# Kamino666/video_features

Measured on NVIDIA H100. Metric: frames/sec CLIP-ViT-B/32 @224px, higher is better.
Workload: dtype f16

## Files before the change

### include/vfeat.h

```cpp
#ifndef VFEAT_H_
#define VFEAT_H_
#include <stddef.h>
#include <stdint.h>

#ifdef __cplusplus
extern "C" {
#endif

#define VF_OK 0
#define VF_ERR_INVALID 1
#define VF_ERR_CUDA 2
#define VF_ERR_NOMEM 3
#define VF_ERR_UNSUPPORTED 4

#define VF_ACT_NONE 0
#define VF_ACT_QUICKGELU 1
#define VF_ACT_RELU 2
#define VF_ACT_SIGMOID 3
#define VF_ACT_TANH 4
#define VF_ACT_LEAKY 5
#define VF_ACT_GELU 6

#define VF_FILTER_BILINEAR 2
#define VF_FILTER_BICUBIC 3

int vf_version(void);
const char* vf_last_error(void);

int vf_sample_indices(const char* method, int param, int64_t frame_cnt, double fps, int64_t* out_idx, int64_t cap,
                      int64_t* out_n);
int vf_shard_range(int64_t n_items, int n_parts, int part, int64_t* begin, int64_t* end);

int vf_resize_u8(const uint8_t* src, int n, int in_h, int in_w, uint8_t* dst, int out_h, int out_w, int filter,
                 uint8_t* tmp, void* stream);
int vf_resize_geometry(int in_h, int in_w, int size, int to_smaller_edge, int* out_h, int* out_w);

int vf_clip_normalize_u8(const uint8_t* src, int n, int src_h, int src_w, float* dst, void* stream);

int vf_gemm_f16(const void* A, int lda, const void* B, int ldb, int M, int N, int K, void* D, int ldd, int out_f32,
                const float* bias, const float* scale, int act, void* stream);
int vf_gemm_f16_accumulate(const void* A, int lda, const void* B, int ldb, int M, int N, int K, float* D, int ldd,
                           const float* bias, const float* scale, int act, void* stream);
int vf_gemm_f16_split(const void* A, int lda, const void* B, int ldb, int M, int N, int K, void* D, int ldd, int split_off,
                      const float* bias, const float* scale, int act, void* stream);
int vf_conv_gemm_f16(const void* X, int C, int64_t P, const void* Wt, int N, int ntaps, int k_per_tap, const int* tap_off,
                     int nsplit, uint64_t lo_mask, int row0, const int* region, void* D, int ldd, int out_f32, int split_off,
                     const float* bias, const float* scale, int act, void* stream);

int vf_gemm_profile(int enable);
int vf_gemm_profile_read(double* ms, int64_t* launches, double* executed_flops);

typedef struct vf_clip_layer_weights {
    const float *ln_1_w, *ln_1_b;
    const float *in_proj_w, *in_proj_b;
    const float *out_proj_w, *out_proj_b;
    const float *ln_2_w, *ln_2_b;
    const float *c_fc_w, *c_fc_b;
    const float *c_proj_w, *c_proj_b;
} vf_clip_layer_weights;

typedef struct vf_clip_weights {
    const float* conv1_w;
    const float* class_embedding;
    const float* positional_embedding;
    const float *ln_pre_w, *ln_pre_b, *ln_post_w, *ln_post_b;
    const float* proj;
    vf_clip_layer_weights layers[12];
} vf_clip_weights;

typedef struct vf_clip vf_clip_t;

int vf_clip_create(vf_clip_t** out, const vf_clip_weights* w, int device, int chunk_frames);
int vf_clip_create_vit(vf_clip_t** out, const vf_clip_weights* w, int device, int chunk_frames, int patch_size);
int vf_clip_destroy(vf_clip_t* h);
int vf_clip_encode_f32(vf_clip_t* h, const float* frames, int n, float* out, void* stream);
int vf_clip_encode_u8(vf_clip_t* h, const uint8_t* frames, int n, int src_h, int src_w, float* out, void* stream);
int vf_clip_encode_u8_host(vf_clip_t* h, const uint8_t* frames_host, int n, int src_h, int src_w, float* out_host,
                           void* stream);
int vf_clip_encode_u8_host_dev(vf_clip_t* h, const uint8_t* frames_host, int n, int src_h, int src_w, float* out_dev,
                               float* out_host, void* stream);

int vf_clip_encode_u8_host_async(vf_clip_t* h, const uint8_t* frames_host, int n, int src_h, int src_w, float* out_dev,
                                 float* out_host, void* stream, int64_t* ticket);
int vf_clip_wait(vf_clip_t* h, int64_t ticket);
int vf_clip_block_attention(vf_clip_t* h, int layer, const void* x, int n_frames, void* out, int fused, void* stream);
int vf_clip_debug_embed_f32(vf_clip_t* h, const float* frames, int n, float* x_out, void* stream);
int vf_clip_debug_embed_u8(vf_clip_t* h, const uint8_t* frames, int n, int src_h, int src_w, float* x_out, void* stream);
int vf_clip_debug_blocks(vf_clip_t* h, float* x, int n_frames, int layer_begin, int layer_end, void* stream);
int vf_clip_debug_head(vf_clip_t* h, const float* x, int n_frames, float* out, void* stream);
int64_t vf_clip_launch_count(const vf_clip_t* h);
int vf_clip_profile(vf_clip_t* h, int enable);
int vf_clip_profile_read(vf_clip_t* h, double* gemm_ms, int64_t* gemm_launches, double* gemm_flops);
int vf_clip_profile_categories(const vf_clip_t* h, double* ms4);

#define VF_I3D_UNITS 57
typedef struct vf_conv_unit {
    const float* w;
    const float *bn_w, *bn_b, *bn_mean, *bn_var;
    int cout, cin, k;
} vf_conv_unit;
typedef struct vf_i3d_weights {
    vf_conv_unit units[VF_I3D_UNITS];
} vf_i3d_weights;
typedef struct vf_i3d vf_i3d_t;

int vf_i3d_create(vf_i3d_t** out, const vf_i3d_weights* w, int in_channels, int device, int max_stacks, int max_T);
int vf_i3d_destroy(vf_i3d_t* h);
int vf_i3d_forward_f32(vf_i3d_t* h, const float* clips, int n, int T, float* out, void* stream);
int vf_i3d_forward_u8(vf_i3d_t* h, const uint8_t* frames, int n, int T, int Hr, int Wr, float* out, void* stream);
int vf_i3d_forward_u8_strided(vf_i3d_t* h, const uint8_t* frames, int n, int T, int64_t stack_stride, int Hr, int Wr,
                              float* out, void* stream);
int vf_i3d_forward_flow(vf_i3d_t* h, const float* flow, int n, int T, int H, int W, float* out, void* stream);
int vf_i3d_read_stage(vf_i3d_t* h, int stage, float* out, int64_t capacity, int* dims5, void* stream);
int64_t vf_i3d_launch_count(const vf_i3d_t* h);
int vf_i3d_conv(const vf_i3d_t* h, int index, int* geom, uint64_t* lo_mask, void* w, float* scale, float* bias);
int vf_i3d_debug_mixed(vf_i3d_t* h, int block, const void* x_pairs, int n, int T, void* out_pairs, void* stream);

typedef struct vf_named_tensor {
    const char* name;
    const float* data;
    int64_t numel;
} vf_named_tensor;
typedef struct vf_raft vf_raft_t;

int vf_raft_create(vf_raft_t** out, const vf_named_tensor* tensors, int n_tensors, int device, int max_frames, int max_h,
                   int max_w);
int vf_raft_destroy(vf_raft_t* h);
int vf_raft_flow(vf_raft_t* h, const void* frames, int is_u8, int chw_layout, int n_frames, int Hs, int Ws, int iters,
                 int unpad, float* out, void* stream);
int vf_raft_padded_size(int Hs, int Ws, int* H, int* W);
int vf_raft_debug_read(vf_raft_t* h, int what, float* out, int64_t capacity, int* dims4, void* stream);
int64_t vf_raft_launch_count(const vf_raft_t* h);
int vf_raft_conv(const vf_raft_t* h, int index, int* geom, uint64_t* lo_mask, void* w, float* scale, float* bias);

typedef struct vf_pwc vf_pwc_t;

int vf_pwc_create(vf_pwc_t** out, const vf_named_tensor* tensors, int n_tensors, int device, int max_frames, int max_h,
                  int max_w);
int vf_pwc_destroy(vf_pwc_t* h);
int vf_pwc_flow(vf_pwc_t* h, const void* frames, int is_u8, int chw_layout, int n_frames, int Hs, int Ws, float* out,
                void* stream);
int vf_pwc_debug_read(vf_pwc_t* h, int what, int level, float* out, int64_t capacity, int* dims4, void* stream);
int64_t vf_pwc_launch_count(const vf_pwc_t* h);
int vf_pwc_conv(const vf_pwc_t* h, int index, int* geom, uint64_t* lo_mask, void* w, float* scale, float* bias);

typedef struct vf_resnet vf_resnet_t;

int vf_resnet_create(vf_resnet_t** out, const vf_named_tensor* tensors, int n_tensors, int depth, int device, int max_frames);
int vf_resnet_destroy(vf_resnet_t* h);
int vf_resnet_forward_f32(vf_resnet_t* h, const float* frames, int n, float* out, void* stream);
int vf_resnet_forward_u8(vf_resnet_t* h, const uint8_t* frames, int n, int Hr, int Wr, float* out, void* stream);
int vf_resnet_read_stage(vf_resnet_t* h, int stage, float* out, int64_t capacity, int* dims4, void* stream);
int64_t vf_resnet_launch_count(const vf_resnet_t* h);
int vf_resnet_conv(const vf_resnet_t* h, int index, int* geom, uint64_t* lo_mask, void* w, float* scale, float* bias);

typedef struct vf_r21d vf_r21d_t;

int vf_r21d_create(vf_r21d_t** out, const vf_named_tensor* tensors, int n_tensors, int device, int max_clips, int max_T);
int vf_r21d_create2(vf_r21d_t** out, const vf_named_tensor* tensors, int n_tensors, int device, int max_clips, int max_T,
                    double bn_eps);
int vf_r21d_destroy(vf_r21d_t* h);
int vf_r21d_forward_f32(vf_r21d_t* h, const float* clips, int n, int T, float* out, void* stream);
int vf_r21d_forward_u8(vf_r21d_t* h, const uint8_t* frames, int n_frames, int H, int W, const int* starts, int n, int T,
                       float* out, void* stream);
int vf_r21d_read_stage(vf_r21d_t* h, int stage, float* out, int64_t capacity, int* dims5, void* stream);
int64_t vf_r21d_launch_count(const vf_r21d_t* h);
int vf_r21d_conv(const vf_r21d_t* h, int index, int* geom, uint64_t* lo_mask, void* w, float* scale, float* bias);

typedef struct vf_clip_rn vf_clip_rn_t;

int vf_clip_rn_create(vf_clip_rn_t** out, const vf_named_tensor* tensors, int n_tensors, int device, int max_frames);
int vf_clip_rn_destroy(vf_clip_rn_t* h);
int vf_clip_rn_info(const vf_clip_rn_t* h, int* info);
int vf_clip_rn_encode_f32(vf_clip_rn_t* h, const float* frames, int n, float* out, void* stream);
int vf_clip_rn_encode_u8(vf_clip_rn_t* h, const uint8_t* frames, int n, int H, int W, float* out, void* stream);
int vf_clip_rn_read_stage(vf_clip_rn_t* h, int stage, float* out, int64_t capacity, int* dims4, void* stream);
int64_t vf_clip_rn_launch_count(const vf_clip_rn_t* h);
int vf_clip_rn_read_pairs(vf_clip_rn_t* h, int stage, void* out, int64_t capacity, void* stream);
int vf_clip_rn_conv(const vf_clip_rn_t* h, int index, int* geom, uint64_t* lo_mask, void* w, float* scale, float* bias);
int vf_clip_rn_debug_block(vf_clip_rn_t* h, int block, const void* x_pairs, int n, void* out_pairs, void* branch_out,
                           void* shortcut_out, void* stream);
int vf_clip_rn_debug_attnpool(vf_clip_rn_t* h, const void* x_pairs, int n, float* features, void* stream);
int vf_clip_rn_debug_attnpool_read(vf_clip_rn_t* h, int what, void* out, int64_t capacity, void* stream);
int vf_debug_clip_rn_attention(const float* kv, const float* q, int n, int T, int E, void* out_pairs, void* stream);

typedef struct vf_clip_vitl vf_clip_vitl_t;

int vf_clip_vitl_create(vf_clip_vitl_t** out, const vf_named_tensor* tensors, int n_tensors, int device, int max_frames);
int vf_clip_vitl_destroy(vf_clip_vitl_t* h);
int vf_clip_vitl_info(const vf_clip_vitl_t* h, int* info);
int vf_clip_vitl_encode_f32(vf_clip_vitl_t* h, const float* frames, int n, float* out, void* stream);
int vf_clip_vitl_encode_u8(vf_clip_vitl_t* h, const uint8_t* frames, int n, int H, int W, float* out, void* stream);
int vf_clip_vitl_debug_embed_f32(vf_clip_vitl_t* h, const float* frames, int n, float* x_out, void* stream);
int vf_clip_vitl_debug_embed_u8(vf_clip_vitl_t* h, const uint8_t* frames, int n, int H, int W, float* x_out,
                                void* stream);
int vf_clip_vitl_debug_blocks(vf_clip_vitl_t* h, float* x, int n, int layer_begin, int layer_end, void* stream);
int vf_clip_vitl_debug_head(vf_clip_vitl_t* h, const float* x, int n, float* out, void* stream);
int vf_clip_vitl_attention(vf_clip_vitl_t* h, const void* qkv, int n_frames, int tokens, void* out, void* stream);
int64_t vf_clip_vitl_launch_count(const vf_clip_vitl_t* h);

typedef struct vf_vggish vf_vggish_t;

int vf_vggish_create(vf_vggish_t** out, const vf_named_tensor* tensors, int n_tensors, const double* hann,
                     const double* mel, const double* interp_win, int n_win, int num_table, int device,
                     int max_examples);
int vf_vggish_destroy(vf_vggish_t* h);
int vf_vggish_forward_pcm16(vf_vggish_t* h, const int16_t* samples, int64_t n_samples, int channels, int sample_rate,
                            float* out, int64_t capacity, int64_t* n_out, void* stream);
int vf_vggish_forward_logmel_f32(vf_vggish_t* h, const float* examples, int n, float* out, void* stream);
int vf_vggish_read_stage(vf_vggish_t* h, int stage, void* out, int64_t capacity, int* dims4, void* stream);
int64_t vf_vggish_launch_count(const vf_vggish_t* h);
int vf_vggish_conv(const vf_vggish_t* h, int index, int* geom, uint64_t* lo_mask, void* w, float* scale, float* bias);
int vf_vggish_time_register(int sample_rate, int64_t t0, int64_t count, double* out);

typedef struct vf_s3d vf_s3d_t;

int vf_s3d_create(vf_s3d_t** out, const vf_named_tensor* tensors, int n_tensors, int device, int max_clips, int max_T);
int vf_s3d_destroy(vf_s3d_t* h);
int vf_s3d_forward_f32(vf_s3d_t* h, const float* clips, int n, int T, float* out, void* stream);
int vf_s3d_forward_u8(vf_s3d_t* h, const uint8_t* frames, int n_frames, int H, int W, const int* starts, int n, int T,
                      float* out, void* stream);
int vf_s3d_read_stage(vf_s3d_t* h, int stage, float* out, int64_t capacity, int* dims5, void* stream);
int64_t vf_s3d_launch_count(const vf_s3d_t* h);
int vf_s3d_conv(const vf_s3d_t* h, int index, int* geom, uint64_t* lo_mask, void* w, float* scale, float* bias);
int vf_s3d_debug_mixed(vf_s3d_t* h, int block, const void* x_pairs, int n, int T, void* out_pairs, void* stream);

#define VF_POOL_GENERAL 0
#define VF_POOL_FAST 1
#define VF_POOL_SAME3 2
int vf_debug_maxpool3d(const void* in, const int* vol_in, void* out, const int* vol_out, int C, const int* k,
                       const int* s, const int* p, int* path, void* stream);
int vf_debug_i3d_head(const void* in, const int* vol, int C, float* out, void* stream);

typedef struct vf_swin3d vf_swin3d_t;

int vf_swin3d_create(vf_swin3d_t** out, const vf_named_tensor* tensors, int n_tensors, int device, int max_clips,
                     int max_T);
int vf_swin3d_destroy(vf_swin3d_t* h);
int vf_swin3d_info(const vf_swin3d_t* h, int* info);
int vf_swin3d_forward_f32(vf_swin3d_t* h, const float* clips, int n, int T, float* out, void* stream);
int vf_swin3d_forward_u8(vf_swin3d_t* h, const uint8_t* frames, int n_frames, int H, int W, const int* starts, int n,
                         int T, float* out, void* stream);
int vf_swin3d_read_stage(vf_swin3d_t* h, int stage, float* out, int64_t capacity, int* dims5, void* stream);
int vf_swin3d_attention(const void* qkv, const float* bias_qkv, const float* table, int n, int Tq, int H, int W, int C,
                        int shifted, void* out, void* stream);
int64_t vf_swin3d_launch_count(const vf_swin3d_t* h);

typedef struct vf_mvit vf_mvit_t;

int vf_mvit_create(vf_mvit_t** out, const vf_named_tensor* tensors, int n_tensors, int device, int max_clips);
int vf_mvit_destroy(vf_mvit_t* h);
int vf_mvit_info(const vf_mvit_t* h, int* info);
int vf_mvit_forward_f32(vf_mvit_t* h, const float* clips, int n, int T, float* out, void* stream);
int vf_mvit_forward_u8(vf_mvit_t* h, const uint8_t* frames, int n_frames, int H, int W, const int* starts, int n, int T,
                       float* out, void* stream);
int vf_mvit_read_stage(vf_mvit_t* h, int stage, float* out, int64_t capacity, int* dims3, void* stream);
int vf_mvit_attention(const void* q, int ldq, const void* k, const void* v, const float* rel_h, const float* rel_w,
                      const float* rel_t, int n, int heads, const int* q_thw, const int* k_thw, int rel, int resid,
                      void* out, void* stream);
int vf_mvit_head_pool(const void* src, int ld_src, int n, int heads, int T, int H, int W, int stride,
                      const float* weight, const float* gamma, const float* beta, void* dst, void* stream);
int vf_mvit_skip_pool(const float* x, int n, int C, int T, int H, int W, float* y, void* stream);
int64_t vf_mvit_launch_count(const vf_mvit_t* h);

typedef struct vf_clip_text vf_clip_text_t;

int vf_clip_text_create(vf_clip_text_t** out, const vf_named_tensor* tensors, int n_tensors, int device, int max_rows);
int vf_clip_text_destroy(vf_clip_text_t* h);
int vf_clip_text_info(const vf_clip_text_t* h, int* info);
int vf_clip_text_encode(vf_clip_text_t* h, const int32_t* tokens, int n, float* out, void* stream);
int vf_clip_text_blocks(vf_clip_text_t* h, float* x, int n, int L, int first, int count, void* stream);
int vf_clip_text_attention(const void* qkv, int n, int L, int heads, void* out, void* stream);
int vf_l2_normalize_rows(const float* x, int n, int C, float* out, void* stream);
int64_t vf_clip_text_launch_count(const vf_clip_text_t* h);

typedef struct vf_dinov2 vf_dinov2_t;

int vf_dinov2_create(vf_dinov2_t** out, const vf_named_tensor* tensors, int n_tensors, int device, int max_frames);
int vf_dinov2_destroy(vf_dinov2_t* h);
int vf_dinov2_info(const vf_dinov2_t* h, int* info);
int vf_dinov2_encode_f32(vf_dinov2_t* h, const float* frames, int n, float* out, void* stream);
int vf_dinov2_encode_u8(vf_dinov2_t* h, const uint8_t* frames, int n, int H, int W, float* out, void* stream);
int vf_dinov2_debug_embed_f32(vf_dinov2_t* h, const float* frames, int n, float* x_out, void* stream);
int vf_dinov2_debug_embed_u8(vf_dinov2_t* h, const uint8_t* frames, int n, int H, int W, float* x_out, void* stream);
int vf_dinov2_debug_blocks(vf_dinov2_t* h, float* x, int n, int layer_begin, int layer_end, void* stream);
int vf_dinov2_debug_head(vf_dinov2_t* h, const float* x, int n, float* out, void* stream);
int vf_dinov2_swiglu(const float* ab, int rows, int hidden, void* out, void* stream);
int vf_dinov2_attention(const void* qkv, int n, int S, int heads, void* out, void* stream);
int64_t vf_dinov2_launch_count(const vf_dinov2_t* h);

typedef struct vf_videomae vf_videomae_t;

int vf_videomae_create(vf_videomae_t** out, const vf_named_tensor* tensors, int n_tensors, const float* config,
                       int device, int max_clips);
int vf_videomae_destroy(vf_videomae_t* h);
int vf_videomae_info(const vf_videomae_t* h, int* info);
int vf_videomae_forward_f32(vf_videomae_t* h, const float* clips, int n, int T, float* out, void* stream);
int vf_videomae_forward_u8(vf_videomae_t* h, const uint8_t* frames, int n_frames, int H, int W, const int* starts, int n,
                           int T, float* out, void* stream);
int vf_videomae_debug_tubelets_u8(vf_videomae_t* h, const uint8_t* frames, int n_frames, int H, int W,
                                  const int* starts, int n, void* tubelets, void* stream);
int vf_videomae_debug_tubelets_f32(vf_videomae_t* h, const float* clips, int n, void* tubelets, void* stream);
int vf_videomae_debug_embed(vf_videomae_t* h, const void* tubelets, int n, float* x_out, void* stream);
int vf_videomae_debug_blocks(vf_videomae_t* h, float* x, int n, int layer_begin, int layer_end, void* stream);
int vf_videomae_debug_head(vf_videomae_t* h, const float* x, int n, float* out, void* stream);
int vf_videomae_debug_drop_lo(vf_videomae_t* h);
int vf_videomae_attention(const void* qkv, int n, int S, int heads, void* out, void* stream);
int64_t vf_videomae_launch_count(const vf_videomae_t* h);

typedef struct vf_head vf_head_t;

int vf_head_create(vf_head_t** out, const float* weight, const float* bias, int n_classes, int n_features, int device);
int vf_head_destroy(vf_head_t* h);
int vf_head_info(const vf_head_t* h, int* n_classes, int* n_features);
int vf_head_forward(vf_head_t* h, const float* feats, int n, int n_features, float* logits, float* probs, int k,
                    int32_t* top_idx, float* top_logit, float* top_prob, void* stream);

#ifdef __cplusplus
}
#endif
#endif
```

### video_features_b200/_lib.py

```python
from __future__ import annotations

import ctypes as C
import os
import threading

_HERE = os.path.dirname(os.path.abspath(__file__))
LIB_PATH = os.environ.get("VF_LIBVFEAT") or os.path.join(_HERE, "libvfeat.so")

VF_OK = 0
VF_ACT_NONE, VF_ACT_QUICKGELU, VF_ACT_RELU, VF_ACT_SIGMOID, VF_ACT_TANH, VF_ACT_LEAKY = 0, 1, 2, 3, 4, 5
VF_ACT_GELU = 6
VF_FILTER_BILINEAR, VF_FILTER_BICUBIC = 2, 3
VF_POOL_GENERAL, VF_POOL_FAST, VF_POOL_SAME3 = 0, 1, 2


class VfError(RuntimeError):
    def __init__(self, code: int, text: str):
        super().__init__(f"libvfeat error {code}: {text}")
        self.code = code


class ClipLayerWeights(C.Structure):
    _fields_ = [(n, C.POINTER(C.c_float)) for n in (
        "ln_1_w", "ln_1_b", "in_proj_w", "in_proj_b", "out_proj_w", "out_proj_b",
        "ln_2_w", "ln_2_b", "c_fc_w", "c_fc_b", "c_proj_w", "c_proj_b")]


class ClipWeights(C.Structure):
    _fields_ = [(n, C.POINTER(C.c_float)) for n in (
        "conv1_w", "class_embedding", "positional_embedding",
        "ln_pre_w", "ln_pre_b", "ln_post_w", "ln_post_b", "proj")] + [("layers", ClipLayerWeights * 12)]


class ConvUnitW(C.Structure):
    _fields_ = [("w", C.POINTER(C.c_float)), ("bn_w", C.POINTER(C.c_float)), ("bn_b", C.POINTER(C.c_float)),
                ("bn_mean", C.POINTER(C.c_float)), ("bn_var", C.POINTER(C.c_float)),
                ("cout", C.c_int), ("cin", C.c_int), ("k", C.c_int)]


I3D_UNITS = 57


class I3DWeights(C.Structure):
    _fields_ = [("units", ConvUnitW * I3D_UNITS)]


class NamedTensor(C.Structure):
    _fields_ = [("name", C.c_char_p), ("data", C.POINTER(C.c_float)), ("numel", C.c_int64)]


def named_tensors(state_dict):
    import numpy as np
    import torch
    items = state_dict.items() if hasattr(state_dict, "items") else state_dict
    items = [(k, v) for k, v in items if torch.is_tensor(v) and v.dtype.is_floating_point]
    keep = []
    arr = (NamedTensor * max(len(items), 1))()
    for i, (k, v) in enumerate(items):
        a = np.ascontiguousarray(v.detach().to("cpu", torch.float32).numpy())
        nm = k.encode()
        keep.append((a, nm))
        arr[i].name = nm
        arr[i].data = a.ctypes.data_as(C.POINTER(C.c_float))
        arr[i].numel = a.size
    return arr, len(items), keep


_lock = threading.Lock()
_lib = None

SIGNATURES = {
    "vf_version": (C.c_int, []),
    "vf_last_error": (C.c_char_p, []),
    "vf_sample_indices": (C.c_int, [C.c_char_p, C.c_int, C.c_int64, C.c_double, C.POINTER(C.c_int64), C.c_int64,
                                    C.POINTER(C.c_int64)]),
    "vf_shard_range": (C.c_int, [C.c_int64, C.c_int, C.c_int, C.POINTER(C.c_int64), C.POINTER(C.c_int64)]),
    "vf_resize_u8": (C.c_int, [C.c_void_p, C.c_int, C.c_int, C.c_int, C.c_void_p, C.c_int, C.c_int, C.c_int,
                               C.c_void_p, C.c_void_p]),
    "vf_resize_geometry": (C.c_int, [C.c_int, C.c_int, C.c_int, C.c_int, C.POINTER(C.c_int), C.POINTER(C.c_int)]),
    "vf_clip_normalize_u8": (C.c_int, [C.c_void_p, C.c_int, C.c_int, C.c_int, C.c_void_p, C.c_void_p]),
    "vf_gemm_f16": (C.c_int, [C.c_void_p, C.c_int, C.c_void_p, C.c_int, C.c_int, C.c_int, C.c_int, C.c_void_p,
                              C.c_int, C.c_int, C.c_void_p, C.c_void_p, C.c_int, C.c_void_p]),
    "vf_gemm_f16_accumulate": (C.c_int, [C.c_void_p, C.c_int, C.c_void_p, C.c_int, C.c_int, C.c_int, C.c_int, C.c_void_p,
                                         C.c_int, C.c_void_p, C.c_void_p, C.c_int, C.c_void_p]),
    "vf_gemm_f16_split": (C.c_int, [C.c_void_p, C.c_int, C.c_void_p, C.c_int, C.c_int, C.c_int, C.c_int, C.c_void_p,
                                    C.c_int, C.c_int, C.c_void_p, C.c_void_p, C.c_int, C.c_void_p]),
    "vf_conv_gemm_f16": (C.c_int, [C.c_void_p, C.c_int, C.c_int64, C.c_void_p, C.c_int, C.c_int, C.c_int,
                                   C.POINTER(C.c_int), C.c_int, C.c_uint64, C.c_int, C.POINTER(C.c_int), C.c_void_p,
                                   C.c_int, C.c_int, C.c_int, C.c_void_p, C.c_void_p, C.c_int, C.c_void_p]),
    "vf_gemm_profile": (C.c_int, [C.c_int]),
    "vf_gemm_profile_read": (C.c_int, [C.POINTER(C.c_double), C.POINTER(C.c_int64), C.POINTER(C.c_double)]),
    "vf_clip_create": (C.c_int, [C.POINTER(C.c_void_p), C.POINTER(ClipWeights), C.c_int, C.c_int]),
    "vf_clip_create_vit": (C.c_int, [C.POINTER(C.c_void_p), C.POINTER(ClipWeights), C.c_int, C.c_int, C.c_int]),
    "vf_clip_destroy": (C.c_int, [C.c_void_p]),
    "vf_clip_encode_f32": (C.c_int, [C.c_void_p, C.c_void_p, C.c_int, C.c_void_p, C.c_void_p]),
    "vf_clip_encode_u8": (C.c_int, [C.c_void_p, C.c_void_p, C.c_int, C.c_int, C.c_int, C.c_void_p, C.c_void_p]),
    "vf_clip_encode_u8_host": (C.c_int, [C.c_void_p, C.c_void_p, C.c_int, C.c_int, C.c_int, C.c_void_p, C.c_void_p]),
    "vf_clip_encode_u8_host_dev": (C.c_int, [C.c_void_p, C.c_void_p, C.c_int, C.c_int, C.c_int, C.c_void_p, C.c_void_p,
                                             C.c_void_p]),
    "vf_clip_encode_u8_host_async": (C.c_int, [C.c_void_p, C.c_void_p, C.c_int, C.c_int, C.c_int, C.c_void_p, C.c_void_p,
                                               C.c_void_p, C.POINTER(C.c_int64)]),
    "vf_clip_wait": (C.c_int, [C.c_void_p, C.c_int64]),
    "vf_clip_block_attention": (C.c_int, [C.c_void_p, C.c_int, C.c_void_p, C.c_int, C.c_void_p, C.c_int, C.c_void_p]),
    "vf_clip_debug_embed_f32": (C.c_int, [C.c_void_p, C.c_void_p, C.c_int, C.c_void_p, C.c_void_p]),
    "vf_clip_debug_embed_u8": (C.c_int, [C.c_void_p, C.c_void_p, C.c_int, C.c_int, C.c_int, C.c_void_p, C.c_void_p]),
    "vf_clip_debug_blocks": (C.c_int, [C.c_void_p, C.c_void_p, C.c_int, C.c_int, C.c_int, C.c_void_p]),
    "vf_clip_debug_head": (C.c_int, [C.c_void_p, C.c_void_p, C.c_int, C.c_void_p, C.c_void_p]),
    "vf_clip_launch_count": (C.c_int64, [C.c_void_p]),
    "vf_i3d_create": (C.c_int, [C.POINTER(C.c_void_p), C.POINTER(I3DWeights), C.c_int, C.c_int, C.c_int, C.c_int]),
    "vf_i3d_destroy": (C.c_int, [C.c_void_p]),
    "vf_i3d_forward_f32": (C.c_int, [C.c_void_p, C.c_void_p, C.c_int, C.c_int, C.c_void_p, C.c_void_p]),
    "vf_i3d_forward_u8": (C.c_int, [C.c_void_p, C.c_void_p, C.c_int, C.c_int, C.c_int, C.c_int, C.c_void_p, C.c_void_p]),
    "vf_i3d_forward_u8_strided": (C.c_int, [C.c_void_p, C.c_void_p, C.c_int, C.c_int, C.c_int64, C.c_int, C.c_int, C.c_void_p,
                                            C.c_void_p]),
    "vf_i3d_forward_flow": (C.c_int, [C.c_void_p, C.c_void_p, C.c_int, C.c_int, C.c_int, C.c_int, C.c_void_p, C.c_void_p]),
    "vf_i3d_read_stage": (C.c_int, [C.c_void_p, C.c_int, C.c_void_p, C.c_int64, C.POINTER(C.c_int), C.c_void_p]),
    "vf_i3d_launch_count": (C.c_int64, [C.c_void_p]),
    "vf_i3d_conv": (C.c_int, [C.c_void_p, C.c_int, C.POINTER(C.c_int), C.POINTER(C.c_uint64), C.c_void_p, C.c_void_p,
                              C.c_void_p]),
    "vf_i3d_debug_mixed": (C.c_int, [C.c_void_p, C.c_int, C.c_void_p, C.c_int, C.c_int, C.c_void_p, C.c_void_p]),
    "vf_raft_create": (C.c_int, [C.POINTER(C.c_void_p), C.POINTER(NamedTensor), C.c_int, C.c_int, C.c_int, C.c_int, C.c_int]),
    "vf_raft_destroy": (C.c_int, [C.c_void_p]),
    "vf_raft_flow": (C.c_int, [C.c_void_p, C.c_void_p, C.c_int, C.c_int, C.c_int, C.c_int, C.c_int, C.c_int, C.c_int,
                               C.c_void_p, C.c_void_p]),
    "vf_raft_padded_size": (C.c_int, [C.c_int, C.c_int, C.POINTER(C.c_int), C.POINTER(C.c_int)]),
    "vf_raft_debug_read": (C.c_int, [C.c_void_p, C.c_int, C.c_void_p, C.c_int64, C.POINTER(C.c_int), C.c_void_p]),
    "vf_raft_launch_count": (C.c_int64, [C.c_void_p]),
    "vf_raft_conv": (C.c_int, [C.c_void_p, C.c_int, C.POINTER(C.c_int), C.POINTER(C.c_uint64), C.c_void_p, C.c_void_p,
                               C.c_void_p]),
    "vf_pwc_create": (C.c_int, [C.POINTER(C.c_void_p), C.POINTER(NamedTensor), C.c_int, C.c_int, C.c_int, C.c_int, C.c_int]),
    "vf_pwc_destroy": (C.c_int, [C.c_void_p]),
    "vf_pwc_flow": (C.c_int, [C.c_void_p, C.c_void_p, C.c_int, C.c_int, C.c_int, C.c_int, C.c_int, C.c_void_p,
                              C.c_void_p]),
    "vf_pwc_debug_read": (C.c_int, [C.c_void_p, C.c_int, C.c_int, C.c_void_p, C.c_int64, C.POINTER(C.c_int), C.c_void_p]),
    "vf_pwc_launch_count": (C.c_int64, [C.c_void_p]),
    "vf_pwc_conv": (C.c_int, [C.c_void_p, C.c_int, C.POINTER(C.c_int), C.POINTER(C.c_uint64), C.c_void_p, C.c_void_p,
                              C.c_void_p]),
    "vf_resnet_create": (C.c_int, [C.POINTER(C.c_void_p), C.POINTER(NamedTensor), C.c_int, C.c_int, C.c_int, C.c_int]),
    "vf_resnet_destroy": (C.c_int, [C.c_void_p]),
    "vf_resnet_forward_f32": (C.c_int, [C.c_void_p, C.c_void_p, C.c_int, C.c_void_p, C.c_void_p]),
    "vf_resnet_forward_u8": (C.c_int, [C.c_void_p, C.c_void_p, C.c_int, C.c_int, C.c_int, C.c_void_p, C.c_void_p]),
    "vf_resnet_read_stage": (C.c_int, [C.c_void_p, C.c_int, C.c_void_p, C.c_int64, C.POINTER(C.c_int), C.c_void_p]),
    "vf_resnet_launch_count": (C.c_int64, [C.c_void_p]),
    "vf_resnet_conv": (C.c_int, [C.c_void_p, C.c_int, C.POINTER(C.c_int), C.POINTER(C.c_uint64), C.c_void_p,
                                 C.c_void_p, C.c_void_p]),
    "vf_r21d_create": (C.c_int, [C.POINTER(C.c_void_p), C.POINTER(NamedTensor), C.c_int, C.c_int, C.c_int, C.c_int]),
    "vf_r21d_create2": (C.c_int, [C.POINTER(C.c_void_p), C.POINTER(NamedTensor), C.c_int, C.c_int, C.c_int, C.c_int,
                                  C.c_double]),
    "vf_r21d_destroy": (C.c_int, [C.c_void_p]),
    "vf_r21d_forward_f32": (C.c_int, [C.c_void_p, C.c_void_p, C.c_int, C.c_int, C.c_void_p, C.c_void_p]),
    "vf_r21d_forward_u8": (C.c_int, [C.c_void_p, C.c_void_p, C.c_int, C.c_int, C.c_int, C.POINTER(C.c_int), C.c_int,
                                     C.c_int, C.c_void_p, C.c_void_p]),
    "vf_r21d_read_stage": (C.c_int, [C.c_void_p, C.c_int, C.c_void_p, C.c_int64, C.POINTER(C.c_int), C.c_void_p]),
    "vf_r21d_launch_count": (C.c_int64, [C.c_void_p]),
    "vf_r21d_conv": (C.c_int, [C.c_void_p, C.c_int, C.POINTER(C.c_int), C.POINTER(C.c_uint64), C.c_void_p,
                               C.c_void_p, C.c_void_p]),
    "vf_s3d_create": (C.c_int, [C.POINTER(C.c_void_p), C.POINTER(NamedTensor), C.c_int, C.c_int, C.c_int, C.c_int]),
    "vf_s3d_destroy": (C.c_int, [C.c_void_p]),
    "vf_s3d_forward_f32": (C.c_int, [C.c_void_p, C.c_void_p, C.c_int, C.c_int, C.c_void_p, C.c_void_p]),
    "vf_s3d_forward_u8": (C.c_int, [C.c_void_p, C.c_void_p, C.c_int, C.c_int, C.c_int, C.POINTER(C.c_int), C.c_int,
                                    C.c_int, C.c_void_p, C.c_void_p]),
    "vf_s3d_read_stage": (C.c_int, [C.c_void_p, C.c_int, C.c_void_p, C.c_int64, C.POINTER(C.c_int), C.c_void_p]),
    "vf_s3d_launch_count": (C.c_int64, [C.c_void_p]),
    "vf_s3d_conv": (C.c_int, [C.c_void_p, C.c_int, C.POINTER(C.c_int), C.POINTER(C.c_uint64), C.c_void_p,
                              C.c_void_p, C.c_void_p]),
    "vf_s3d_debug_mixed": (C.c_int, [C.c_void_p, C.c_int, C.c_void_p, C.c_int, C.c_int, C.c_void_p, C.c_void_p]),
    "vf_debug_maxpool3d": (C.c_int, [C.c_void_p, C.POINTER(C.c_int), C.c_void_p, C.POINTER(C.c_int), C.c_int,
                                     C.POINTER(C.c_int), C.POINTER(C.c_int), C.POINTER(C.c_int), C.POINTER(C.c_int),
                                     C.c_void_p]),
    "vf_debug_i3d_head": (C.c_int, [C.c_void_p, C.POINTER(C.c_int), C.c_int, C.c_void_p, C.c_void_p]),
    "vf_clip_rn_create": (C.c_int, [C.POINTER(C.c_void_p), C.POINTER(NamedTensor), C.c_int, C.c_int, C.c_int]),
    "vf_clip_rn_destroy": (C.c_int, [C.c_void_p]),
    "vf_clip_rn_info": (C.c_int, [C.c_void_p, C.POINTER(C.c_int)]),
    "vf_clip_rn_encode_f32": (C.c_int, [C.c_void_p, C.c_void_p, C.c_int, C.c_void_p, C.c_void_p]),
    "vf_clip_rn_encode_u8": (C.c_int, [C.c_void_p, C.c_void_p, C.c_int, C.c_int, C.c_int, C.c_void_p, C.c_void_p]),
    "vf_clip_rn_read_stage": (C.c_int, [C.c_void_p, C.c_int, C.c_void_p, C.c_int64, C.POINTER(C.c_int), C.c_void_p]),
    "vf_clip_rn_launch_count": (C.c_int64, [C.c_void_p]),
    "vf_clip_rn_conv": (C.c_int, [C.c_void_p, C.c_int, C.POINTER(C.c_int), C.POINTER(C.c_uint64), C.c_void_p,
                                  C.c_void_p, C.c_void_p]),
    "vf_clip_rn_read_pairs": (C.c_int, [C.c_void_p, C.c_int, C.c_void_p, C.c_int64, C.c_void_p]),
    "vf_clip_rn_debug_block": (C.c_int, [C.c_void_p, C.c_int, C.c_void_p, C.c_int, C.c_void_p, C.c_void_p, C.c_void_p,
                                         C.c_void_p]),
    "vf_clip_rn_debug_attnpool": (C.c_int, [C.c_void_p, C.c_void_p, C.c_int, C.c_void_p, C.c_void_p]),
    "vf_clip_rn_debug_attnpool_read": (C.c_int, [C.c_void_p, C.c_int, C.c_void_p, C.c_int64, C.c_void_p]),
    "vf_debug_clip_rn_attention": (C.c_int, [C.c_void_p, C.c_void_p, C.c_int, C.c_int, C.c_int, C.c_void_p,
                                             C.c_void_p]),
    "vf_swin3d_create": (C.c_int, [C.POINTER(C.c_void_p), C.POINTER(NamedTensor), C.c_int, C.c_int, C.c_int, C.c_int]),
    "vf_swin3d_destroy": (C.c_int, [C.c_void_p]),
    "vf_swin3d_info": (C.c_int, [C.c_void_p, C.POINTER(C.c_int)]),
    "vf_swin3d_forward_f32": (C.c_int, [C.c_void_p, C.c_void_p, C.c_int, C.c_int, C.c_void_p, C.c_void_p]),
    "vf_swin3d_forward_u8": (C.c_int, [C.c_void_p, C.c_void_p, C.c_int, C.c_int, C.c_int, C.POINTER(C.c_int), C.c_int,
                                       C.c_int, C.c_void_p, C.c_void_p]),
    "vf_swin3d_read_stage": (C.c_int, [C.c_void_p, C.c_int, C.c_void_p, C.c_int64, C.POINTER(C.c_int), C.c_void_p]),
    "vf_swin3d_attention": (C.c_int, [C.c_void_p, C.c_void_p, C.c_void_p, C.c_int, C.c_int, C.c_int, C.c_int, C.c_int,
                                      C.c_int, C.c_void_p, C.c_void_p]),
    "vf_swin3d_launch_count": (C.c_int64, [C.c_void_p]),
    "vf_mvit_create": (C.c_int, [C.POINTER(C.c_void_p), C.POINTER(NamedTensor), C.c_int, C.c_int, C.c_int]),
    "vf_mvit_destroy": (C.c_int, [C.c_void_p]),
    "vf_mvit_info": (C.c_int, [C.c_void_p, C.POINTER(C.c_int)]),
    "vf_mvit_forward_f32": (C.c_int, [C.c_void_p, C.c_void_p, C.c_int, C.c_int, C.c_void_p, C.c_void_p]),
    "vf_mvit_forward_u8": (C.c_int, [C.c_void_p, C.c_void_p, C.c_int, C.c_int, C.c_int, C.POINTER(C.c_int), C.c_int,
                                     C.c_int, C.c_void_p, C.c_void_p]),
    "vf_mvit_read_stage": (C.c_int, [C.c_void_p, C.c_int, C.c_void_p, C.c_int64, C.POINTER(C.c_int), C.c_void_p]),
    "vf_mvit_attention": (C.c_int, [C.c_void_p, C.c_int, C.c_void_p, C.c_void_p, C.c_void_p, C.c_void_p, C.c_void_p,
                                    C.c_int, C.c_int, C.POINTER(C.c_int), C.POINTER(C.c_int), C.c_int, C.c_int,
                                    C.c_void_p, C.c_void_p]),
    "vf_mvit_head_pool": (C.c_int, [C.c_void_p, C.c_int, C.c_int, C.c_int, C.c_int, C.c_int, C.c_int, C.c_int,
                                    C.c_void_p, C.c_void_p, C.c_void_p, C.c_void_p, C.c_void_p]),
    "vf_mvit_skip_pool": (C.c_int, [C.c_void_p, C.c_int, C.c_int, C.c_int, C.c_int, C.c_int, C.c_void_p, C.c_void_p]),
    "vf_mvit_launch_count": (C.c_int64, [C.c_void_p]),
    "vf_clip_vitl_create": (C.c_int, [C.POINTER(C.c_void_p), C.POINTER(NamedTensor), C.c_int, C.c_int, C.c_int]),
    "vf_clip_vitl_destroy": (C.c_int, [C.c_void_p]),
    "vf_clip_vitl_info": (C.c_int, [C.c_void_p, C.POINTER(C.c_int)]),
    "vf_clip_vitl_encode_f32": (C.c_int, [C.c_void_p, C.c_void_p, C.c_int, C.c_void_p, C.c_void_p]),
    "vf_clip_vitl_encode_u8": (C.c_int, [C.c_void_p, C.c_void_p, C.c_int, C.c_int, C.c_int, C.c_void_p, C.c_void_p]),
    "vf_clip_vitl_debug_embed_f32": (C.c_int, [C.c_void_p, C.c_void_p, C.c_int, C.c_void_p, C.c_void_p]),
    "vf_clip_vitl_debug_embed_u8": (C.c_int, [C.c_void_p, C.c_void_p, C.c_int, C.c_int, C.c_int, C.c_void_p,
                                              C.c_void_p]),
    "vf_clip_vitl_debug_blocks": (C.c_int, [C.c_void_p, C.c_void_p, C.c_int, C.c_int, C.c_int, C.c_void_p]),
    "vf_clip_vitl_debug_head": (C.c_int, [C.c_void_p, C.c_void_p, C.c_int, C.c_void_p, C.c_void_p]),
    "vf_clip_vitl_attention": (C.c_int, [C.c_void_p, C.c_void_p, C.c_int, C.c_int, C.c_void_p, C.c_void_p]),
    "vf_clip_vitl_launch_count": (C.c_int64, [C.c_void_p]),
    "vf_vggish_create": (C.c_int, [C.POINTER(C.c_void_p), C.POINTER(NamedTensor), C.c_int, C.c_void_p, C.c_void_p,
                                   C.c_void_p, C.c_int, C.c_int, C.c_int, C.c_int]),
    "vf_vggish_destroy": (C.c_int, [C.c_void_p]),
    "vf_vggish_forward_pcm16": (C.c_int, [C.c_void_p, C.c_void_p, C.c_int64, C.c_int, C.c_int, C.c_void_p, C.c_int64,
                                          C.POINTER(C.c_int64), C.c_void_p]),
    "vf_vggish_forward_logmel_f32": (C.c_int, [C.c_void_p, C.c_void_p, C.c_int, C.c_void_p, C.c_void_p]),
    "vf_vggish_read_stage": (C.c_int, [C.c_void_p, C.c_int, C.c_void_p, C.c_int64, C.POINTER(C.c_int), C.c_void_p]),
    "vf_vggish_launch_count": (C.c_int64, [C.c_void_p]),
    "vf_vggish_conv": (C.c_int, [C.c_void_p, C.c_int, C.POINTER(C.c_int), C.POINTER(C.c_uint64), C.c_void_p,
                                 C.c_void_p, C.c_void_p]),
    "vf_vggish_time_register": (C.c_int, [C.c_int, C.c_int64, C.c_int64, C.c_void_p]),
    "vf_clip_text_create": (C.c_int, [C.POINTER(C.c_void_p), C.POINTER(NamedTensor), C.c_int, C.c_int, C.c_int]),
    "vf_clip_text_destroy": (C.c_int, [C.c_void_p]),
    "vf_clip_text_info": (C.c_int, [C.c_void_p, C.POINTER(C.c_int)]),
    "vf_clip_text_encode": (C.c_int, [C.c_void_p, C.c_void_p, C.c_int, C.c_void_p, C.c_void_p]),
    "vf_clip_text_blocks": (C.c_int, [C.c_void_p, C.c_void_p, C.c_int, C.c_int, C.c_int, C.c_int, C.c_void_p]),
    "vf_clip_text_attention": (C.c_int, [C.c_void_p, C.c_int, C.c_int, C.c_int, C.c_void_p, C.c_void_p]),
    "vf_l2_normalize_rows": (C.c_int, [C.c_void_p, C.c_int, C.c_int, C.c_void_p, C.c_void_p]),
    "vf_clip_text_launch_count": (C.c_int64, [C.c_void_p]),
    "vf_dinov2_create": (C.c_int, [C.POINTER(C.c_void_p), C.POINTER(NamedTensor), C.c_int, C.c_int, C.c_int]),
    "vf_dinov2_destroy": (C.c_int, [C.c_void_p]),
    "vf_dinov2_info": (C.c_int, [C.c_void_p, C.POINTER(C.c_int)]),
    "vf_dinov2_encode_f32": (C.c_int, [C.c_void_p, C.c_void_p, C.c_int, C.c_void_p, C.c_void_p]),
    "vf_dinov2_encode_u8": (C.c_int, [C.c_void_p, C.c_void_p, C.c_int, C.c_int, C.c_int, C.c_void_p, C.c_void_p]),
    "vf_dinov2_debug_embed_f32": (C.c_int, [C.c_void_p, C.c_void_p, C.c_int, C.c_void_p, C.c_void_p]),
    "vf_dinov2_debug_embed_u8": (C.c_int, [C.c_void_p, C.c_void_p, C.c_int, C.c_int, C.c_int, C.c_void_p, C.c_void_p]),
    "vf_dinov2_debug_blocks": (C.c_int, [C.c_void_p, C.c_void_p, C.c_int, C.c_int, C.c_int, C.c_void_p]),
    "vf_dinov2_debug_head": (C.c_int, [C.c_void_p, C.c_void_p, C.c_int, C.c_void_p, C.c_void_p]),
    "vf_dinov2_swiglu": (C.c_int, [C.c_void_p, C.c_int, C.c_int, C.c_void_p, C.c_void_p]),
    "vf_dinov2_attention": (C.c_int, [C.c_void_p, C.c_int, C.c_int, C.c_int, C.c_void_p, C.c_void_p]),
    "vf_dinov2_launch_count": (C.c_int64, [C.c_void_p]),
    "vf_videomae_create": (C.c_int, [C.POINTER(C.c_void_p), C.POINTER(NamedTensor), C.c_int, C.POINTER(C.c_float),
                                     C.c_int, C.c_int]),
    "vf_videomae_destroy": (C.c_int, [C.c_void_p]),
    "vf_videomae_info": (C.c_int, [C.c_void_p, C.POINTER(C.c_int)]),
    "vf_videomae_forward_f32": (C.c_int, [C.c_void_p, C.c_void_p, C.c_int, C.c_int, C.c_void_p, C.c_void_p]),
    "vf_videomae_forward_u8": (C.c_int, [C.c_void_p, C.c_void_p, C.c_int, C.c_int, C.c_int, C.POINTER(C.c_int), C.c_int,
                                         C.c_int, C.c_void_p, C.c_void_p]),
    "vf_videomae_debug_tubelets_u8": (C.c_int, [C.c_void_p, C.c_void_p, C.c_int, C.c_int, C.c_int, C.POINTER(C.c_int),
                                                C.c_int, C.c_void_p, C.c_void_p]),
    "vf_videomae_debug_tubelets_f32": (C.c_int, [C.c_void_p, C.c_void_p, C.c_int, C.c_void_p, C.c_void_p]),
    "vf_videomae_debug_embed": (C.c_int, [C.c_void_p, C.c_void_p, C.c_int, C.c_void_p, C.c_void_p]),
    "vf_videomae_debug_blocks": (C.c_int, [C.c_void_p, C.c_void_p, C.c_int, C.c_int, C.c_int, C.c_void_p]),
    "vf_videomae_debug_head": (C.c_int, [C.c_void_p, C.c_void_p, C.c_int, C.c_void_p, C.c_void_p]),
    "vf_videomae_debug_drop_lo": (C.c_int, [C.c_void_p]),
    "vf_videomae_attention": (C.c_int, [C.c_void_p, C.c_int, C.c_int, C.c_int, C.c_void_p, C.c_void_p]),
    "vf_videomae_launch_count": (C.c_int64, [C.c_void_p]),
    "vf_head_create": (C.c_int, [C.POINTER(C.c_void_p), C.c_void_p, C.c_void_p, C.c_int, C.c_int, C.c_int]),
    "vf_head_destroy": (C.c_int, [C.c_void_p]),
    "vf_head_info": (C.c_int, [C.c_void_p, C.POINTER(C.c_int), C.POINTER(C.c_int)]),
    "vf_head_forward": (C.c_int, [C.c_void_p, C.c_void_p, C.c_int, C.c_int, C.c_void_p, C.c_void_p, C.c_int, C.c_void_p,
                                  C.c_void_p, C.c_void_p, C.c_void_p]),
    "vf_clip_profile": (C.c_int, [C.c_void_p, C.c_int]),
    "vf_clip_profile_categories": (C.c_int, [C.c_void_p, C.POINTER(C.c_double)]),
    "vf_clip_profile_read": (C.c_int, [C.c_void_p, C.POINTER(C.c_double), C.POINTER(C.c_int64),
                                       C.POINTER(C.c_double)]),
}


def lib() -> C.CDLL:
    global _lib
    if _lib is None:
        with _lock:
            if _lib is None:
                if not os.path.exists(LIB_PATH):
                    raise FileNotFoundError(
                        f"{LIB_PATH} not found: build the CUDA extension first (__graft_entry__.build()). "
                        "There is no CPU fallback.")
                l = C.CDLL(LIB_PATH)
                for name, (res, args) in SIGNATURES.items():
                    fn = getattr(l, name)
                    fn.restype = res
                    fn.argtypes = args
                _lib = l
    return _lib


def check(status: int) -> None:
    if status != VF_OK:
        raise VfError(status, lib().vf_last_error().decode("utf-8", "replace"))


def read_conv(fn, handle, index: int, device):
    import torch
    geom = (C.c_int * 15)()
    mask = C.c_uint64()
    check(fn(handle, index, geom, C.byref(mask), None, None, None))
    n_out, ntaps, kpt = geom[0], geom[1], geom[2]
    w = torch.empty((n_out, 2 * ntaps * kpt), dtype=torch.float16, device=device)
    scale = torch.empty(n_out, dtype=torch.float32, device=device)
    bias = torch.empty(n_out, dtype=torch.float32, device=device)
    check(fn(handle, index, geom, C.byref(mask), w.data_ptr(), scale.data_ptr(), bias.data_ptr()))
    shifts = [tuple(geom[3 + 3 * j:6 + 3 * j]) for j in range(ntaps)]
    return dict(n_out=n_out, ntaps=ntaps, k_per_tap=kpt, shifts=shifts, lo_mask=mask.value, w=w, scale=scale, bias=bias)


MIXED_SIDE = (28, 28, 14, 14, 14, 14, 14, 7, 7)
MIXED_WIDTHS = ((192, 64, 128, 32, 32), (256, 128, 192, 96, 64), (480, 192, 208, 48, 64), (512, 160, 224, 64, 64),
                (512, 128, 256, 64, 64), (512, 112, 288, 64, 64), (528, 256, 320, 128, 128), (832, 256, 320, 128, 128),
                (832, 384, 384, 128, 128))


def debug_mixed(fn, handle, block: int, x, device):
    import torch
    if not 0 <= block < len(MIXED_SIDE):
        raise ValueError(f"Mixed block {block} outside 0 .. {len(MIXED_SIDE) - 1}")
    S, cin, cout = MIXED_SIDE[block], MIXED_WIDTHS[block][0], sum(MIXED_WIDTHS[block][1:])
    if x.dtype != torch.float16 or x.dim() != 5 or tuple(x.shape[2:]) != (S + 2, S + 2, 2 * cin) or x.shape[1] < 3:
        raise ValueError(f"block {block} takes an fp16 pair volume (n, T + 2, {S + 2}, {S + 2}, {2 * cin}), T >= 1; "
                         f"got {x.dtype} {tuple(x.shape)}")
    if x.device != torch.device(device):
        raise ValueError(f"the volume is on {x.device}, the engine on {device}")
    x = x.contiguous()
    out = torch.empty(tuple(x.shape[:4]) + (2 * cout,), dtype=torch.float16, device=device)
    with torch.cuda.device(device):
        check(fn(handle, block, x.data_ptr(), x.shape[0], x.shape[1] - 2, out.data_ptr(),
                 torch.cuda.current_stream().cuda_stream))
    return out


def debug_maxpool3d(x, vol_in, vol_out, channels: int, k, s, p):
    import torch
    assert x.dtype == torch.float16 and x.is_cuda
    assert x.numel() == vol_in[0] * vol_in[1] * vol_in[2] * vol_in[3] * 2 * channels, (x.shape, vol_in, channels)
    x = x.contiguous()
    out = torch.empty(tuple(vol_out[:4]) + (2 * channels,), dtype=torch.float16, device=x.device)
    path = C.c_int(-1)
    with torch.cuda.device(x.device):
        check(lib().vf_debug_maxpool3d(x.data_ptr(), (C.c_int * 10)(*vol_in), out.data_ptr(), (C.c_int * 10)(*vol_out),
                                       channels, (C.c_int * 3)(*k), (C.c_int * 3)(*s), (C.c_int * 3)(*p), C.byref(path),
                                       torch.cuda.current_stream().cuda_stream))
    return out, path.value


def debug_i3d_head(x, vol, channels: int):
    import torch
    assert x.dtype == torch.float16 and x.is_cuda
    assert x.numel() == vol[0] * vol[1] * vol[2] * vol[3] * 2 * channels, (x.shape, vol, channels)
    x = x.contiguous()
    out = torch.empty((vol[0], channels), dtype=torch.float32, device=x.device)
    with torch.cuda.device(x.device):
        check(lib().vf_debug_i3d_head(x.data_ptr(), (C.c_int * 10)(*vol), channels, out.data_ptr(),
                                      torch.cuda.current_stream().cuda_stream))
    return out


def debug_clip_rn_attention(kv, q):
    import torch
    if kv.dtype != torch.float32 or q.dtype != torch.float32 or kv.dim() != 3 or q.dim() != 2:
        raise ValueError(f"kv (n, T, 2E) and q (n, E) fp32; got {kv.dtype} {tuple(kv.shape)}, {q.dtype} {tuple(q.shape)}")
    n, T, E2 = kv.shape
    if E2 % 2 or tuple(q.shape) != (n, E2 // 2):
        raise ValueError(f"kv {tuple(kv.shape)} and q {tuple(q.shape)} do not agree on (n, E)")
    if not kv.is_cuda or q.device != kv.device:
        raise ValueError(f"kv on {kv.device}, q on {q.device}: both must be on one CUDA device")
    kv, q = kv.contiguous(), q.contiguous()
    out = torch.empty((n, E2), dtype=torch.float16, device=kv.device)
    with torch.cuda.device(kv.device):
        check(lib().vf_debug_clip_rn_attention(kv.data_ptr(), q.data_ptr(), n, T, E2 // 2, out.data_ptr(),
                                               torch.cuda.current_stream().cuda_stream))
    return out


def read_split_conv(fn, handle, index: int, device):
    import torch
    geom = (C.c_int * 196)()
    mask = C.c_uint64()
    check(fn(handle, index, geom, C.byref(mask), None, None, None))
    n_out, ntaps, kpt, nsplit = geom[0], geom[1], geom[2], geom[3]
    w = torch.empty((n_out, nsplit * ntaps * kpt), dtype=torch.float16, device=device)
    scale = torch.empty(n_out, dtype=torch.float32, device=device)
    bias = torch.empty(n_out, dtype=torch.float32, device=device)
    check(fn(handle, index, geom, C.byref(mask), w.data_ptr(), scale.data_ptr(), bias.data_ptr()))
    shifts = [tuple(geom[4 + 3 * j:7 + 3 * j]) for j in range(ntaps)]
    return dict(n_out=n_out, ntaps=ntaps, k_per_tap=kpt, nsplit=nsplit, shifts=shifts, lo_mask=mask.value, w=w,
                scale=scale, bias=bias)
```

### video_features_b200/csrc/gemm.cu

```cuda
#include "gemm_kernel.cuh"

namespace vf {

extern template int launch_bn<1, false, true>(GEMM_LAUNCH_ARGS);
extern template int launch_bn<1, true, true>(GEMM_LAUNCH_ARGS);
extern template int launch_bn<1, false, false>(GEMM_LAUNCH_ARGS);
extern template int launch_bn<1, true, false>(GEMM_LAUNCH_ARGS);
extern template int launch_bn<2, false, false>(GEMM_LAUNCH_ARGS);
extern template int launch_bn<2, true, false>(GEMM_LAUNCH_ARGS);

namespace {

typedef CUresult (*EncodeTiledFn)(CUtensorMap*, CUtensorMapDataType, cuuint32_t, void*, const cuuint64_t*,
                                  const cuuint64_t*, const cuuint32_t*, const cuuint32_t*, CUtensorMapInterleave,
                                  CUtensorMapSwizzle, CUtensorMapL2promotion, CUtensorMapFloatOOBfill);

EncodeTiledFn get_encode_tiled() {
    static EncodeTiledFn fn = nullptr;
    if (fn) return fn;
    void* p = nullptr;
    cudaDriverEntryPointQueryResult q;
    if (cudaGetDriverEntryPoint("cuTensorMapEncodeTiled", &p, cudaEnableDefault, &q) != cudaSuccess ||
        q != cudaDriverEntryPointSuccess)
        return nullptr;
    fn = reinterpret_cast<EncodeTiledFn>(p);
    return fn;
}

}

int device_sm_count() {
    static std::atomic<int> sms[64];
    int dev = 0;
    if (cudaGetDevice(&dev) != cudaSuccess || dev < 0 || dev >= 64) return 132;
    int v = sms[dev].load(std::memory_order_relaxed);
    if (v == 0) {
        if (cudaDeviceGetAttribute(&v, cudaDevAttrMultiProcessorCount, dev) != cudaSuccess || v <= 0) v = 132;
        sms[dev].store(v, std::memory_order_relaxed);
    }
    return v;
}

int make_tmap_2d(CUtensorMap* out, const void* base, int elem_bytes, uint64_t rows, uint64_t cols,
                 uint64_t row_pitch_bytes, uint32_t box_rows, uint32_t box_cols) {
    EncodeTiledFn enc = get_encode_tiled();
    if (!enc) return fail(VF_ERR_CUDA, "cuTensorMapEncodeTiled entry point unavailable (no CUDA driver?)");
    if ((reinterpret_cast<uintptr_t>(base) & 15) || (row_pitch_bytes & 15))
        return fail(VF_ERR_INVALID, "TMA operand must be 16-byte aligned with a 16-byte multiple row pitch");
    if (box_cols * uint32_t(elem_bytes) != 128) return fail(VF_ERR_INVALID, "TMA box rows must be 128 bytes");
    const CUtensorMapDataType dt = elem_bytes == 2 ? CU_TENSOR_MAP_DATA_TYPE_FLOAT16 : CU_TENSOR_MAP_DATA_TYPE_FLOAT32;
    cuuint64_t dims[2] = {cols, rows};
    cuuint64_t strides[1] = {row_pitch_bytes};
    cuuint32_t box[2] = {box_cols, box_rows};
    cuuint32_t estr[2] = {1, 1};
    CUresult r = enc(out, dt, 2, const_cast<void*>(base), dims, strides, box, estr, CU_TENSOR_MAP_INTERLEAVE_NONE,
                     CU_TENSOR_MAP_SWIZZLE_128B, CU_TENSOR_MAP_L2_PROMOTION_L2_256B, CU_TENSOR_MAP_FLOAT_OOB_FILL_NONE);
    if (r != CUDA_SUCCESS) return fail(VF_ERR_CUDA, "cuTensorMapEncodeTiled failed with CUresult %d", int(r));
    return VF_OK;
}

struct GemmProf {
    bool on = false;
    std::vector<cudaEvent_t> ev;
    size_t used = 0;
    double flops = 0.0;
};
static thread_local GemmProf g_prof;

template <bool PP>
static int run_gemm_launch(const CUtensorMap& tmA, const CUtensorMap& tmB, const CUtensorMap& tmD,
                           const CUtensorMap& tmD2, int bn, const GemmEpi& ep, int M, int N, const ConvGeom& cg,
                           cudaStream_t stream) {
    const bool split = ep.split_off > 0 && !ep.out_f32;
    if constexpr (!PP) {
        if (cg.nsplit == 2)
            return split ? launch_bn<2, true, PP>(tmA, tmB, tmD, tmD2, bn, ep, M, N, cg, stream)
                         : launch_bn<2, false, PP>(tmA, tmB, tmD, tmD2, bn, ep, M, N, cg, stream);
    }
    return split ? launch_bn<1, true, PP>(tmA, tmB, tmD, tmD2, bn, ep, M, N, cg, stream)
                 : launch_bn<1, false, PP>(tmA, tmB, tmD, tmD2, bn, ep, M, N, cg, stream);
}

static int run_gemm(const CUtensorMap& tmA, bool pp, const __half* B, int ldb, int64_t Ktot, int M, int N,
                    const ConvGeom& cg, const GemmEpi& ep, cudaStream_t stream) {
    if (!ep.out) return fail(VF_ERR_INVALID, "gemm: null output");
    if (reinterpret_cast<uintptr_t>(ep.out) & 15) return fail(VF_ERR_INVALID, "gemm: output must be 16-byte aligned");
    if (ep.accumulate && !ep.out_f32) return fail(VF_ERR_INVALID, "gemm: accumulate needs fp32 output");
    if (N % 8) return fail(VF_ERR_INVALID, "gemm: N=%d must be a multiple of 8", N);
    if (ep.act < VF_ACT_NONE || ep.act > VF_ACT_GELU) return fail(VF_ERR_INVALID, "gemm: unknown activation %d", ep.act);
    if (ep.out_f32 ? (ep.ldo % 4) : (ep.ldo % 8)) return fail(VF_ERR_INVALID, "gemm: ldo breaks 16-byte rows");
    if (ep.split_off && (ep.out_f32 || ep.split_off < N || ep.split_off % 8))
        return fail(VF_ERR_INVALID, "gemm: split output needs fp16 out and split_off >= N, multiple of 8");
    const int bm = tile_rows(pp);
    const int64_t num_m = (M + bm - 1) / bm, sms = device_sm_count();
    int bn = 256;
    int64_t best = INT64_MAX;
    for (int cand : {256, 192, 128, 64}) {
        const int64_t cost = (num_m * ((N + cand - 1) / cand) + sms - 1) / sms * cand;
        if (cost < best) { best = cost; bn = cand; }
    }
    CUtensorMap tmB, tmD, tmD2;
    VF_TRY(make_tmap_2d(&tmB, B, 2, uint64_t(N), uint64_t(Ktot), uint64_t(ldb) * 2, uint32_t(bn), BK));
    const int eb = ep.out_f32 ? 4 : 2;
    VF_TRY(make_tmap_2d(&tmD, ep.out, eb, uint64_t(M), uint64_t(N), uint64_t(ep.ldo) * eb, EPI_ROWS, 128 / eb));
    if (ep.split_off)
        VF_TRY(make_tmap_2d(&tmD2, static_cast<__half*>(ep.out) + ep.split_off, eb, uint64_t(M), uint64_t(N),
                            uint64_t(ep.ldo) * eb, EPI_ROWS, 128 / eb));
    else
        tmD2 = tmD;
    auto launch = [&] {
        return pp ? run_gemm_launch<true>(tmA, tmB, tmD, tmD2, bn, ep, M, N, cg, stream)
                  : run_gemm_launch<false>(tmA, tmB, tmD, tmD2, bn, ep, M, N, cg, stream);
    };
    if (!g_prof.on) return launch();
    if (g_prof.used + 2 > g_prof.ev.size())
        for (int i = 0; i < 2; ++i) {
            cudaEvent_t e;
            VF_CUDA(cudaEventCreate(&e));
            g_prof.ev.push_back(e);
        }
    VF_CUDA(cudaEventRecord(g_prof.ev[g_prof.used], stream));
    const int st = launch();
    VF_CUDA(cudaEventRecord(g_prof.ev[g_prof.used + 1], stream));
    g_prof.used += 2;
    double kexec = double(Ktot);
    if (cg.nsplit == 2 && cg.lo_mask) {
        const int kpt = (cg.k_per_tap + BK - 1) / BK;
        int skipped = 0;
        for (int kk = 0; kk < kpt && kk < 64; ++kk) skipped += int((cg.lo_mask >> kk) & 1ull);
        kexec -= double(cg.ntaps) * skipped * BK;
    }
    g_prof.flops += 2.0 * double(M) * double(N) * kexec;
    return st;
}

bool gemm_profile_on() { return g_prof.on; }
int gemm_profile(int enable) {
    g_prof.on = enable != 0;
    return VF_OK;
}
int gemm_profile_read(double* ms, int64_t* launches, double* flops) {
    VF_CUDA(cudaDeviceSynchronize());
    double t = 0.0;
    for (size_t i = 0; i + 1 < g_prof.used; i += 2) {
        float x = 0.f;
        VF_CUDA(cudaEventElapsedTime(&x, g_prof.ev[i], g_prof.ev[i + 1]));
        t += x;
    }
    if (ms) *ms = t;
    if (launches) *launches = int64_t(g_prof.used / 2);
    if (flops) *flops = g_prof.flops;
    g_prof.used = 0;
    g_prof.flops = 0.0;
    return VF_OK;
}

int gemm_f16(const __half* A, int lda, const __half* B, int ldb, int M, int N, int K, const GemmEpi& ep,
             cudaStream_t stream) {
    if (M <= 0 || N <= 0 || K <= 0) return fail(VF_ERR_INVALID, "gemm: empty problem %dx%dx%d", M, N, K);
    if (K % 8 || lda % 8 || ldb % 8) return fail(VF_ERR_INVALID, "gemm: K/lda/ldb must be multiples of 8");
    ConvGeom cg;
    memset(&cg, 0, sizeof(cg));
    cg.ntaps = 1;
    cg.k_per_tap = K;
    cg.nsplit = 1;
    CUtensorMap tmA;
    VF_TRY(make_tmap_2d(&tmA, A, 2, uint64_t(M), uint64_t(K), uint64_t(lda) * 2, tile_rows(true), BK));
    return run_gemm(tmA, true, B, ldb, K, M, N, cg, ep, stream);
}

int conv_gemm_f16(const __half* X, int C, int64_t P, const __half* Wt, int N, const ConvGeom& g, const GemmEpi& ep,
                  cudaStream_t stream) {
    if (P <= 0 || P > 0x7fffffff || N <= 0 || C <= 0) return fail(VF_ERR_INVALID, "conv_gemm: bad size");
    if (C % 8) return fail(VF_ERR_INVALID, "conv_gemm: C=%d must be a multiple of 8", C);
    if (g.ntaps < 1 || g.ntaps > 64 || g.k_per_tap < 8 || g.k_per_tap % 8)
        return fail(VF_ERR_INVALID, "conv_gemm: bad tap geometry (%d taps x %d)", g.ntaps, g.k_per_tap);
    if (g.nsplit != 1 && g.nsplit != 2) return fail(VF_ERR_INVALID, "conv_gemm: nsplit must be 1 or 2");
    const int kpt = (g.k_per_tap + BK - 1) / BK;
    if (g.lo_mask && (kpt > 64 || (kpt < 64 && (g.lo_mask >> kpt) != 0)))
        return fail(VF_ERR_INVALID, "conv_gemm: lo_mask 0x%llx names K blocks beyond the %d of a tap", g.lo_mask, kpt);
    if (g.mask && (g.Tp < 1 || g.Hp < 1 || g.Wp < 1 || g.row0 < 0))
        return fail(VF_ERR_INVALID, "conv_gemm: bad mask volume %dx%dx%d, row0 %d", g.Tp, g.Hp, g.Wp, g.row0);
    CUtensorMap tmA;
    VF_TRY(make_tmap_2d(&tmA, X, 2, uint64_t(P), uint64_t(g.k_per_tap), uint64_t(C) * 2, tile_rows(false), BK));
    const int64_t Ktot = int64_t(g.ntaps) * g.k_per_tap * g.nsplit;
    if (Ktot % 8) return fail(VF_ERR_INVALID, "conv_gemm: K must be a multiple of 8");
    return run_gemm(tmA, false, Wt, int(Ktot), Ktot, int(P), N, g, ep, stream);
}

}
```

### video_features_b200/csrc/gemm_kernel.cuh

```cuda
#pragma once
#include <stdarg.h>
#include <stdlib.h>
#include <string.h>

#include <atomic>
#include <vector>

#include "common.cuh"
#include "internal.h"
#include "wgmma.cuh"

namespace vf {

namespace {

constexpr int BK = 64;
constexpr int THREADS = 384;
constexpr uint32_t PRODUCER_REGS = 40, CONSUMER_REGS = 232;
constexpr int EPI_ROWS = 64;
constexpr uint32_t STG_BYTES = EPI_ROWS * 128;
constexpr uint32_t STAGING_BYTES = 2 * 2 * STG_BYTES;
constexpr uint32_t SMEM_LIMIT = 227 * 1024;
constexpr uint32_t MAX_STAGES = 8;
constexpr uint32_t RING_BUDGET = SMEM_LIMIT - STAGING_BYTES - 2 * MAX_STAGES * 8 - 1024;

template <int BN, int NSPLIT, bool PP>
struct GemmCfg {
    static constexpr int BM = PP ? 64 : 128;
    static constexpr uint32_t A_BYTES = BM * BK * 2;
    static constexpr uint32_t B_TILE = BN * BK * 2;
    static constexpr uint32_t B_BYTES = NSPLIT * B_TILE;
    static constexpr uint32_t STAGE_BYTES = A_BYTES + B_BYTES;
    static constexpr int STAGES = RING_BUDGET / STAGE_BYTES > MAX_STAGES ? MAX_STAGES : int(RING_BUDGET / STAGE_BYTES);
    static constexpr uint32_t BAR_BYTES = 2 * STAGES * 8;
    static constexpr uint32_t SMEM_BYTES = STAGES * STAGE_BYTES + STAGING_BYTES + BAR_BYTES + 1024;
    static_assert(STAGES >= 2, "at least two pipeline stages");
    static_assert(SMEM_BYTES <= SMEM_LIMIT, "shared memory budget");
    static_assert(A_BYTES % 1024 == 0 && B_TILE % 1024 == 0, "swizzle-128B tiles must stay 1024-byte aligned");
};

constexpr int tile_rows(bool pp) { return pp ? GemmCfg<64, 1, true>::BM : GemmCfg<64, 1, false>::BM; }

template <int ACT>
__device__ __forceinline__ float apply_act(float v) {
    if (ACT == VF_ACT_QUICKGELU) {
        return __fdividef(v, 1.0f + __expf(-1.702f * v));
    } else if (ACT == VF_ACT_RELU) {
        return fmaxf(v, 0.0f);
    } else if (ACT == VF_ACT_SIGMOID) {
        return __fdividef(1.0f, 1.0f + __expf(-v));
    } else if (ACT == VF_ACT_TANH) {
        return 1.0f - __fdividef(2.0f, 1.0f + __expf(2.0f * v));
    } else if (ACT == VF_ACT_LEAKY) {
        return v > 0.0f ? v : __fmul_rn(v, 0.1f);
    } else if (ACT == VF_ACT_GELU) {
        return 0.5f * v * (1.0f + erff(v * 0.70710678118654752f));
    }
    return v;
}

template <int BN, int NSPLIT, bool SPLIT, bool PP, int ACT>
__global__ void __launch_bounds__(THREADS, 1)
gemm_f16_kernel(const __grid_constant__ CUtensorMap tmA, const __grid_constant__ CUtensorMap tmB,
                const __grid_constant__ CUtensorMap tmD, const __grid_constant__ CUtensorMap tmD2, const GemmEpi ep,
                const int M, const int N, const __grid_constant__ ConvGeom cg) {
    using Cfg = GemmCfg<BN, NSPLIT, PP>;
    static_assert(PP ? NSPLIT == 1 : true, "split weights run in the conv mode only");
    constexpr int STAGES = Cfg::STAGES;
    constexpr int BM = Cfg::BM;
    extern __shared__ uint8_t smem_raw[];
    uint8_t* smem = reinterpret_cast<uint8_t*>((reinterpret_cast<uintptr_t>(smem_raw) + 1023) & ~uintptr_t(1023));
    uint8_t* sA = smem;
    uint8_t* sB = smem + STAGES * Cfg::A_BYTES;
    uint8_t* sD = smem + STAGES * Cfg::STAGE_BYTES;
    uint64_t* full = reinterpret_cast<uint64_t*>(sD + STAGING_BYTES);
    uint64_t* empty = full + STAGES;

    const int warp = threadIdx.x >> 5;
    const int lane = threadIdx.x & 31;
    const int num_m = (M + BM - 1) / BM;
    const int num_n = (N + BN - 1) / BN;
    const int num_tiles = num_m * num_n;
    auto tile_m0 = [&](int tile) { return (PP ? tile / num_n : tile % num_m) * BM; };
    auto tile_n0 = [&](int tile) { return (PP ? tile % num_n : tile / num_m) * BN; };
    const int cta_tiles = (num_tiles - 1 - int(blockIdx.x)) / int(gridDim.x) + 1;
    const int kpt = (cg.k_per_tap + BK - 1) / BK;
    const int num_k = cg.ntaps * kpt;

    if (threadIdx.x == 0) {
        tma_prefetch_desc(&tmA);
        tma_prefetch_desc(&tmB);
        tma_prefetch_desc(&tmD);
        if (SPLIT) tma_prefetch_desc(&tmD2);
        for (int i = 0; i < STAGES; ++i) {
            mbar_init(&full[i], 1);
            mbar_init(&empty[i], PP ? 4 : 8);
        }
        fence_mbar_init();
    }
    __syncthreads();

    if (warp < 4) {
        setmaxnreg_dec<PRODUCER_REGS>();
        if (warp == 0 && lane == 0) {
            int stage = 0;
            uint32_t phase = 0;
            for (int i = 0; i < cta_tiles; ++i) {
                const int tile = blockIdx.x + i * gridDim.x;
                const int m0 = tile_m0(tile), n0 = tile_n0(tile);
                for (int tap = 0; tap < cg.ntaps; ++tap) {
                    const int arow = m0 + cg.tap_off[tap];
                    const int bcol = tap * cg.k_per_tap;
                    for (int kk = 0; kk < kpt; ++kk) {
                        mbar_wait(&empty[stage], phase ^ 1);
                        const bool lo_blk = NSPLIT == 2 && ((cg.lo_mask >> kk) & 1ull);
                        mbar_expect_tx(&full[stage], Cfg::A_BYTES + (lo_blk ? Cfg::B_TILE : Cfg::B_BYTES));
                        tma_load_2d(sA + stage * Cfg::A_BYTES, &tmA, &full[stage], kk * BK, arow);
                        tma_load_2d(sB + stage * Cfg::B_BYTES, &tmB, &full[stage], bcol + kk * BK, n0);
                        if (NSPLIT == 2 && !lo_blk)
                            tma_load_2d(sB + stage * Cfg::B_BYTES + Cfg::B_TILE, &tmB, &full[stage],
                                        cg.ntaps * cg.k_per_tap + bcol + kk * BK, n0);
                        if (++stage == STAGES) { stage = 0; phase ^= 1; }
                    }
                }
            }
        }
        return;
    }

    setmaxnreg_inc<CONSUMER_REGS>();
    const int wg = (warp >> 2) - 1;
    const int wq = warp & 3;
    constexpr int R = BN / 2;
    float acc[R];
    const bool issuer = (threadIdx.x & 127) == 0;
    uint32_t buf = 0;
    auto wg_sync = [&] {
        if (wg == 0) named_bar_sync(1, 128);
        else named_bar_sync(2, 128);
    };
    auto store_subtile = [&](int col, int row) {
        fence_proxy_async();
        if (issuer) bulk_wait_read<0>();
        wg_sync();
        if (issuer) {
            const uint8_t* src = sD + (wg * 2 + buf) * STG_BYTES;
            if (ep.accumulate) tma_reduce_add_2d(&tmD, src, col, row);
            else tma_store_2d(&tmD, src, col, row);
            bulk_commit();
        }
        buf ^= 1;
    };
    auto wait_turn = [&] {
        if (wg == 0) named_bar_sync(3, 256);
        else named_bar_sync(4, 256);
    };
    auto pass_turn = [&] {
        if (wg == 0) named_bar_arrive(4, 256);
        else named_bar_arrive(3, 256);
    };
    for (int i = PP ? wg : 0; i < cta_tiles; i += PP ? 2 : 1) {
        const int tile = blockIdx.x + i * gridDim.x;
        const int m0 = tile_m0(tile) + (PP ? 0 : wg * 64), n0 = tile_n0(tile);
        const uint64_t first = uint64_t(i) * uint64_t(num_k);
        int stage = int(first % STAGES);
        uint32_t phase = uint32_t(first / STAGES) & 1u;
        if (PP && i > 0) wait_turn();
        int prev = -1;
        for (int kb = 0, kk = 0; kb < num_k; ++kb) {
            mbar_wait(&full[stage], phase);
            const uint64_t adesc = wgmma_desc_sw128(sA + stage * Cfg::A_BYTES + (PP ? 0 : wg * (64 * 128)));
            const uint64_t bdesc = wgmma_desc_sw128(sB + stage * Cfg::B_BYTES);
            const bool lo_blk = NSPLIT == 2 && ((cg.lo_mask >> kk) & 1ull);
            wgmma_fence_regs<R>(acc);
            wgmma_fence();
#pragma unroll
            for (int k = 0; k < BK / 16; ++k) {
                Wgmma<BN>::mma(acc, adesc + 2 * k, bdesc + 2 * k, (kb | k) != 0 ? 1u : 0u);
                if (NSPLIT == 2 && !lo_blk) Wgmma<BN>::mma(acc, adesc + 2 * k, bdesc + (Cfg::B_TILE >> 4) + 2 * k, 1u);
            }
            wgmma_commit();
            wgmma_wait<1>();
            wgmma_fence_regs<R>(acc);
            if (prev >= 0) {
                __syncwarp();
                if (lane == 0) mbar_arrive(&empty[prev]);
            }
            prev = stage;
            if (++stage == STAGES) { stage = 0; phase ^= 1; }
            if (++kk == kpt) kk = 0;
        }
        if (PP && i + 1 < cta_tiles) pass_turn();
        float2 sc[8], bi[8];
        auto load_sb = [&](int s) {
#pragma unroll
            for (int c = 0; c < 8; ++c) {
                const int n = min(n0 + 64 * s + 8 * c + 2 * (lane & 3), N - 2);
                sc[c] = ep.scale ? __ldg(reinterpret_cast<const float2*>(ep.scale + n)) : make_float2(1.f, 1.f);
                bi[c] = ep.bias ? __ldg(reinterpret_cast<const float2*>(ep.bias + n)) : make_float2(-0.f, -0.f);
            }
        };
        load_sb(0);
        wgmma_wait<0>();
        wgmma_fence_regs<R>(acc);
        __syncwarp();
        if (lane == 0) mbar_arrive(&empty[prev]);

        bool keep[2] = {true, true};
        if (cg.mask) {
#pragma unroll
            for (int h = 0; h < 2; ++h) {
                const int mm = m0 + wq * 16 + (lane >> 2) + 8 * h - cg.row0;
                const int w = mm % cg.Wp, r1 = mm / cg.Wp;
                const int hh = r1 % cg.Hp, r2 = r1 / cg.Hp;
                const int tt = r2 % cg.Tp;
                keep[h] = (mm >= 0) && (w >= cg.w0) && (w < cg.w1) && (hh >= cg.h0) && (hh < cg.h1) && (tt >= cg.t0) && (tt < cg.t1);
            }
        }
        const int row = m0;
        const uint32_t stg = smem_u32(sD) + wg * 2 * STG_BYTES + (wq * 16 + (lane >> 2)) * 128;
        const int swz = lane >> 2;
#pragma unroll
        for (int s = 0; s < BN / 64; ++s) {
            if (n0 + 64 * s >= N) break;
#pragma unroll
            for (int c = 0; c < 8; ++c)
#pragma unroll
                for (int h = 0; h < 2; ++h) {
                    const int j = 8 * s + c;
                    float v0 = __fadd_rn(__fmul_rn(acc[4 * j + 2 * h], sc[c].x), bi[c].x);
                    float v1 = __fadd_rn(__fmul_rn(acc[4 * j + 2 * h + 1], sc[c].y), bi[c].y);
                    v0 = apply_act<ACT>(v0);
                    v1 = apply_act<ACT>(v1);
                    acc[4 * j + 2 * h] = keep[h] ? v0 : 0.f;
                    acc[4 * j + 2 * h + 1] = keep[h] ? v1 : 0.f;
                }
            if (s + 1 < BN / 64) load_sb(s + 1);
            if (SPLIT) {
                if (issuer) bulk_wait_read<0>();
                wg_sync();
#pragma unroll
                for (int c = 0; c < 8; ++c)
#pragma unroll
                    for (int h = 0; h < 2; ++h) {
                        const int j = 8 * s + c;
                        const float v0 = acc[4 * j + 2 * h], v1 = acc[4 * j + 2 * h + 1];
                        const __half2 hi = __floats2half2_rn(v0, v1);
                        const uint32_t off = h * 8 * 128 + ((c ^ swz) << 4) + 4 * (lane & 3);
                        st_shared_b32(stg + off, *reinterpret_cast<const uint32_t*>(&hi));
                        st_shared_b32(stg + STG_BYTES + off, pack_half2(v0 - __low2float(hi), v1 - __high2float(hi)));
                    }
                fence_proxy_async();
                wg_sync();
                if (issuer) {
                    tma_store_2d(&tmD, sD + wg * 2 * STG_BYTES, n0 + 64 * s, row);
                    tma_store_2d(&tmD2, sD + (wg * 2 + 1) * STG_BYTES, n0 + 64 * s, row);
                    bulk_commit();
                }
            } else if (ep.out_f32) {
#pragma unroll
                for (int q = 0; q < 2; ++q) {
                    if (q == 1 && n0 + 64 * s + 32 >= N) break;
                    const uint32_t d = stg + buf * STG_BYTES;
#pragma unroll
                    for (int c = 0; c < 4; ++c) {
                        const int j = 8 * s + 4 * q + c;
                        const int chunk = 2 * c + ((lane & 3) >> 1);
#pragma unroll
                        for (int h = 0; h < 2; ++h)
                            st_shared_v2_f32(d + h * 8 * 128 + ((chunk ^ swz) << 4) + 8 * (lane & 1), acc[4 * j + 2 * h],
                                             acc[4 * j + 2 * h + 1]);
                    }
                    store_subtile(n0 + 64 * s + 32 * q, row);
                }
            } else {
                const uint32_t d = stg + buf * STG_BYTES;
#pragma unroll
                for (int c = 0; c < 8; ++c)
#pragma unroll
                    for (int h = 0; h < 2; ++h) {
                        const int j = 8 * s + c;
                        st_shared_b32(d + h * 8 * 128 + ((c ^ swz) << 4) + 4 * (lane & 3),
                                      pack_half2(acc[4 * j + 2 * h], acc[4 * j + 2 * h + 1]));
                    }
                store_subtile(n0 + 64 * s, row);
            }
        }
    }
    if (issuer) bulk_wait<0>();
}

template <int BN, int NSPLIT, bool SPLIT, bool PP, int ACT>
int launch_gemm(const CUtensorMap& tmA, const CUtensorMap& tmB, const CUtensorMap& tmD, const CUtensorMap& tmD2,
                const GemmEpi& ep, int M, int N, const ConvGeom& cg, cudaStream_t stream) {
    using Cfg = GemmCfg<BN, NSPLIT, PP>;
    static std::atomic<bool> attr_set[64];
    int dev = 0;
    VF_CUDA(cudaGetDevice(&dev));
    if (dev < 0 || dev >= 64 || !attr_set[dev].load(std::memory_order_acquire)) {
        VF_CUDA(cudaFuncSetAttribute(gemm_f16_kernel<BN, NSPLIT, SPLIT, PP, ACT>,
                                     cudaFuncAttributeMaxDynamicSharedMemorySize, Cfg::SMEM_BYTES));
        if (dev >= 0 && dev < 64) attr_set[dev].store(true, std::memory_order_release);
    }
    const int tiles = ((M + Cfg::BM - 1) / Cfg::BM) * ((N + BN - 1) / BN);
    const int sms = device_sm_count();
    const int grid = tiles < sms ? tiles : sms;
    gemm_f16_kernel<BN, NSPLIT, SPLIT, PP, ACT><<<grid, THREADS, Cfg::SMEM_BYTES, stream>>>(tmA, tmB, tmD, tmD2, ep, M,
                                                                                            N, cg);
    VF_CUDA(cudaGetLastError());
    return VF_OK;
}

template <int BN, int NSPLIT, bool SPLIT, bool PP>
int launch_act(const CUtensorMap& tmA, const CUtensorMap& tmB, const CUtensorMap& tmD, const CUtensorMap& tmD2,
               const GemmEpi& ep, int M, int N, const ConvGeom& cg, cudaStream_t stream) {
    switch (ep.act) {
        case VF_ACT_QUICKGELU:
            return launch_gemm<BN, NSPLIT, SPLIT, PP, VF_ACT_QUICKGELU>(tmA, tmB, tmD, tmD2, ep, M, N, cg, stream);
        case VF_ACT_RELU:
            return launch_gemm<BN, NSPLIT, SPLIT, PP, VF_ACT_RELU>(tmA, tmB, tmD, tmD2, ep, M, N, cg, stream);
        case VF_ACT_SIGMOID:
            return launch_gemm<BN, NSPLIT, SPLIT, PP, VF_ACT_SIGMOID>(tmA, tmB, tmD, tmD2, ep, M, N, cg, stream);
        case VF_ACT_TANH:
            return launch_gemm<BN, NSPLIT, SPLIT, PP, VF_ACT_TANH>(tmA, tmB, tmD, tmD2, ep, M, N, cg, stream);
        case VF_ACT_LEAKY:
            if constexpr (NSPLIT == 2 && !PP)
                return launch_gemm<BN, NSPLIT, SPLIT, PP, VF_ACT_LEAKY>(tmA, tmB, tmD, tmD2, ep, M, N, cg, stream);
            else
                return fail(VF_ERR_INVALID, "gemm: LeakyReLU is built for split-weight convolutions (nsplit = 2) only");
        case VF_ACT_GELU:
            if constexpr (!SPLIT && ((NSPLIT == 1 && PP) || (NSPLIT == 2 && !PP)))
                return launch_gemm<BN, NSPLIT, SPLIT, PP, VF_ACT_GELU>(tmA, tmB, tmD, tmD2, ep, M, N, cg, stream);
            else
                return fail(VF_ERR_INVALID, "gemm: GELU is built for gemm_f16 and split-weight convolutions, without split output, only");
        default:
            return launch_gemm<BN, NSPLIT, SPLIT, PP, VF_ACT_NONE>(tmA, tmB, tmD, tmD2, ep, M, N, cg, stream);
    }
}

}

#define GEMM_LAUNCH_ARGS                                                                                           \
    const CUtensorMap &tmA, const CUtensorMap &tmB, const CUtensorMap &tmD, const CUtensorMap &tmD2, int bn,       \
        const GemmEpi &ep, int M, int N, const ConvGeom &cg, cudaStream_t stream
template <int NSPLIT, bool SPLIT, bool PP>
int launch_bn(GEMM_LAUNCH_ARGS) {
    if (bn == 256) return launch_act<256, NSPLIT, SPLIT, PP>(tmA, tmB, tmD, tmD2, ep, M, N, cg, stream);
    if (bn == 192) return launch_act<192, NSPLIT, SPLIT, PP>(tmA, tmB, tmD, tmD2, ep, M, N, cg, stream);
    if (bn == 128) return launch_act<128, NSPLIT, SPLIT, PP>(tmA, tmB, tmD, tmD2, ep, M, N, cg, stream);
    return launch_act<64, NSPLIT, SPLIT, PP>(tmA, tmB, tmD, tmD2, ep, M, N, cg, stream);
}

}
```

### video_features_b200/csrc/host.cu

```cuda
#include <math.h>
#include <stdarg.h>
#include <stdlib.h>
#include <string.h>

#include <map>
#include <mutex>
#include <string>
#include <tuple>
#include <vector>

#include "internal.h"

namespace vf {

static thread_local char g_err[1024] = {0};

void set_error(const char* fmt, ...) {
    va_list ap;
    va_start(ap, fmt);
    vsnprintf(g_err, sizeof(g_err), fmt, ap);
    va_end(ap);
}
int fail(int code, const char* fmt, ...) {
    va_list ap;
    va_start(ap, fmt);
    vsnprintf(g_err, sizeof(g_err), fmt, ap);
    va_end(ap);
    return code;
}

static double filter_bicubic(double x) {
    const double a = -0.5;
    if (x < 0.0) x = -x;
    if (x < 1.0) return ((a + 2.0) * x - (a + 3.0)) * x * x + 1;
    if (x < 2.0) return (((x - 5) * x + 8) * x - 4) * a;
    return 0.0;
}
static double filter_bilinear(double x) {
    if (x < 0.0) x = -x;
    if (x < 1.0) return 1.0 - x;
    return 0.0;
}

struct CoefTable {
    int ksize = 0;
    std::vector<int> bounds;
    std::vector<int> coefs;
};

static bool build_coeffs(int in_size, int out_size, int filter, CoefTable* t) {
    double (*f)(double);
    double fsupport;
    if (filter == VF_FILTER_BICUBIC) { f = filter_bicubic; fsupport = 2.0; }
    else if (filter == VF_FILTER_BILINEAR) { f = filter_bilinear; fsupport = 1.0; }
    else return false;
    const double scale = double(in_size) / double(out_size);
    double filterscale = scale;
    if (filterscale < 1.0) filterscale = 1.0;
    const double support = fsupport * filterscale;
    const int ksize = int(ceil(support)) * 2 + 1;
    t->ksize = ksize;
    t->bounds.assign(size_t(out_size) * 2, 0);
    t->coefs.assign(size_t(out_size) * ksize, 0);
    std::vector<double> k(ksize);
    const double ss = 1.0 / filterscale;
    for (int xx = 0; xx < out_size; ++xx) {
        const double center = (xx + 0.5) * scale;
        double ww = 0.0;
        int xmin = int(center - support + 0.5);
        if (xmin < 0) xmin = 0;
        int xmax = int(center + support + 0.5);
        if (xmax > in_size) xmax = in_size;
        xmax -= xmin;
        for (int x = 0; x < xmax; ++x) {
            const double w = f((x + xmin - center + 0.5) * ss);
            k[x] = w;
            ww += w;
        }
        for (int x = 0; x < xmax; ++x) {
            if (ww != 0.0) k[x] /= ww;
        }
        for (int x = 0; x < xmax; ++x) {
            const double v = k[x];
            t->coefs[size_t(xx) * ksize + x] = v < 0 ? int(-0.5 + v * double(1 << 22)) : int(0.5 + v * double(1 << 22));
        }
        t->bounds[2 * xx] = xmin;
        t->bounds[2 * xx + 1] = xmax;
    }
    return true;
}

struct DevCoefs {
    int ksize = 0;
    int* bounds = nullptr;
    int* coefs = nullptr;
};
static std::mutex g_coef_mu;
static std::map<std::tuple<int, int, int, int>, DevCoefs> g_coef_cache;

static int get_dev_coefs(int in_size, int out_size, int filter, cudaStream_t s, DevCoefs* out) {
    int dev = 0;
    VF_CUDA(cudaGetDevice(&dev));
    std::lock_guard<std::mutex> lk(g_coef_mu);
    auto key = std::make_tuple(dev, in_size, out_size, filter);
    auto it = g_coef_cache.find(key);
    if (it != g_coef_cache.end()) { *out = it->second; return VF_OK; }
    CoefTable t;
    if (!build_coeffs(in_size, out_size, filter, &t)) return fail(VF_ERR_INVALID, "resize: unknown filter %d", filter);
    DevCoefs d;
    d.ksize = t.ksize;
    VF_CUDA(cudaMalloc(&d.bounds, t.bounds.size() * sizeof(int)));
    VF_CUDA(cudaMalloc(&d.coefs, t.coefs.size() * sizeof(int)));
    VF_CUDA(cudaMemcpy(d.bounds, t.bounds.data(), t.bounds.size() * sizeof(int), cudaMemcpyHostToDevice));
    VF_CUDA(cudaMemcpy(d.coefs, t.coefs.data(), t.coefs.size() * sizeof(int), cudaMemcpyHostToDevice));
    (void)s;
    g_coef_cache[key] = d;
    *out = d;
    return VF_OK;
}

int resize_u8(const uint8_t* src, int n, int in_h, int in_w, uint8_t* dst, int out_h, int out_w, int filter,
              uint8_t* tmp, cudaStream_t s) {
    if (n <= 0) return VF_OK;
    if (in_h <= 0 || in_w <= 0 || out_h <= 0 || out_w <= 0) return fail(VF_ERR_INVALID, "resize: bad geometry");
    DevCoefs kh, kv;
    VF_TRY(get_dev_coefs(in_w, out_w, filter, s, &kh));
    VF_TRY(get_dev_coefs(in_h, out_h, filter, s, &kv));
    if (out_w != in_w && out_h != in_h && tmp == nullptr) return fail(VF_ERR_INVALID, "resize: tmp scratch required");
    return launch_resample(src, n, in_h, in_w, tmp, dst, out_h, out_w, kh.bounds, kh.coefs, kh.ksize, kv.bounds,
                           kv.coefs, kv.ksize, s);
}

int center_crop_offset(int dim, int crop) {
    const int d = dim - crop;
    if (d >= 0) {
        if ((d & 1) == 0) return d / 2;
        const int q = d / 2;
        return (q & 1) ? q + 1 : q;
    }
    const int e = -d;
    if ((e & 1) == 0) return -(e / 2);
    const int q = e / 2;
    return -((q & 1) ? q + 1 : q);
}

int check_device(int device) {
    VF_CUDA(cudaSetDevice(device));
    int major = 0, minor = 0;
    VF_CUDA(cudaDeviceGetAttribute(&major, cudaDevAttrComputeCapabilityMajor, device));
    VF_CUDA(cudaDeviceGetAttribute(&minor, cudaDevAttrComputeCapabilityMinor, device));
    if (major != 9 || minor != 0)
        return fail(VF_ERR_UNSUPPORTED, "device %d is sm_%d%d; this library is built for sm_90a only", device, major, minor);
    return VF_OK;
}

bool graphs_enabled() {
    const char* e = getenv("VF_NO_GRAPH");
    return !(e && e[0] == '1');
}

bool graph_trace() {
    const char* e = getenv("VF_GRAPH_TRACE");
    return e && e[0] == '1';
}

int engine_alloc(EngineCore* h, void** p, size_t bytes) {
    void* q = nullptr;
    bytes += 65536;
    cudaError_t e = cudaMalloc(&q, bytes);
    if (e != cudaSuccess) return fail(VF_ERR_NOMEM, "%s: cudaMalloc(%zu bytes): %s", h->who, bytes, cudaGetErrorString(e));
    h->allocs.push_back(q);
    VF_CUDA(cudaMemset(q, 0, bytes));
    *p = q;
    return VF_OK;
}

int open_stream(EngineCore* h) {
    VF_CUDA(cudaStreamCreateWithFlags(&h->cs, cudaStreamNonBlocking));
    VF_CUDA(cudaEventCreateWithFlags(&h->ev_in, cudaEventDisableTiming));
    VF_CUDA(cudaEventCreateWithFlags(&h->ev_out, cudaEventDisableTiming));
    return VF_OK;
}

int enter(EngineCore* h, cudaStream_t user) {
    VF_CUDA(cudaSetDevice(h->device));
    VF_CUDA(cudaEventRecord(h->ev_in, user));
    VF_CUDA(cudaStreamWaitEvent(h->cs, h->ev_in, 0));
    return VF_OK;
}

int leave(EngineCore* h, cudaStream_t user) {
    VF_CUDA(cudaEventRecord(h->ev_out, h->cs));
    VF_CUDA(cudaStreamWaitEvent(user, h->ev_out, 0));
    return VF_OK;
}

void release(EngineCore* h) {
    cudaSetDevice(h->device);
    cudaDeviceSynchronize();
    for (void* p : h->allocs) cudaFree(p);
    for (auto& kv : h->graphs) cudaGraphExecDestroy(kv.second.exec);
    cudaFree(h->resized);
    cudaFree(h->resize_tmp);
    if (h->cs) cudaStreamDestroy(h->cs);
    if (h->ev_in) cudaEventDestroy(h->ev_in);
    if (h->ev_out) cudaEventDestroy(h->ev_out);
}

int grow(EngineCore* h, uint8_t** p, size_t* cap, size_t need) {
    if (need <= *cap) return VF_OK;
    if (*p) {
        VF_CUDA(cudaStreamSynchronize(h->cs));
        VF_CUDA(cudaFree(*p));
        *p = nullptr; *cap = 0;
    }
    void* q = nullptr;
    const cudaError_t e = cudaMalloc(&q, need);
    if (e != cudaSuccess) return fail(VF_ERR_NOMEM, "%s: cudaMalloc(%zu bytes): %s", h->who, need, cudaGetErrorString(e));
    *p = static_cast<uint8_t*>(q);
    *cap = need;
    return VF_OK;
}

int upload_f32(EngineCore* h, float** dst, const float* src, size_t count) {
    if (!src) return fail(VF_ERR_INVALID, "%s: missing weight tensor", h->who);
    VF_TRY(ralloc(h, dst, count));
    VF_CUDA(cudaMemcpy(*dst, src, count * sizeof(float), cudaMemcpyHostToDevice));
    return VF_OK;
}

int upload_f16(EngineCore* h, __half** dst, const float* src, size_t rows, size_t cols, size_t ld, bool transpose) {
    if (!src) return fail(VF_ERR_INVALID, "%s: missing weight tensor", h->who);
    if (ld == 0) ld = cols;
    std::vector<__half> tmp(rows * ld, __float2half_rn(0.f));
    for (size_t r = 0; r < rows; ++r)
        for (size_t c = 0; c < cols; ++c) tmp[r * ld + c] = __float2half_rn(transpose ? src[c * rows + r] : src[r * cols + c]);
    VF_TRY(ralloc(h, dst, rows * ld));
    VF_CUDA(cudaMemcpy(*dst, tmp.data(), tmp.size() * sizeof(__half), cudaMemcpyHostToDevice));
    return VF_OK;
}

int capture_graph(EngineCore* h, cudaStream_t s, const std::function<int()>& run, CachedGraph* g) {
    const int64_t before = h->launches;
    cudaGraph_t graph = nullptr;
    VF_CUDA(cudaStreamBeginCapture(s, cudaStreamCaptureModeRelaxed));
    const int st = run();
    const cudaError_t ce = cudaStreamEndCapture(s, &graph);
    g->launches = h->launches - before;
    h->launches = before;
    if (st != VF_OK) { if (graph) cudaGraphDestroy(graph); return st; }
    if (ce != cudaSuccess) return fail(VF_ERR_CUDA, "cudaStreamEndCapture: %s", cudaGetErrorString(ce));
    const cudaError_t ie = cudaGraphInstantiate(&g->exec, graph, 0);
    cudaGraphDestroy(graph);
    if (ie != cudaSuccess) return fail(VF_ERR_CUDA, "cudaGraphInstantiate: %s", cudaGetErrorString(ie));
    return VF_OK;
}

int run_graphed(EngineCore* h, const GraphKey& key, const std::function<int()>& run) {
    if (!h->use_graph || gemm_profile_on()) return run();
    auto it = h->graphs.find(key);
    if (it == h->graphs.end()) {
        const bool full = h->graphs.size() >= h->max_graphs;
        if (h->seen.size() > 4096) h->seen.clear();
        if (++h->seen[key] < h->capture_after || (full && !h->evict_when_full)) return run();
        CachedGraph g;
        VF_TRY(capture_graph(h, h->cs, run, &g));
        if (full) {
            cudaGraphExecDestroy(h->graphs.begin()->second.exec);
            h->graphs.erase(h->graphs.begin());
        }
        it = h->graphs.emplace(key, g).first;
        if (h->trace_graphs)
            fprintf(stderr, "[vf] %s: graph captured for key (%d, %d, %d, %d), %zu cached\n", h->who, key[0], key[1], key[2],
                    key[3], h->graphs.size());
    }
    VF_CUDA(cudaGraphLaunch(it->second.exec, h->cs));
    h->launches += it->second.launches;
    return VF_OK;
}

int frame_geometry(const char* who, int H, int W, int resize_to, int crop, FrameGeom* g) {
    if (H <= 0 || W <= 0) return fail(VF_ERR_INVALID, "%s: bad frame geometry %dx%d", who, H, W);
    VF_TRY(vf_resize_geometry(H, W, resize_to, 1, &g->rh, &g->rw));
    if (g->rh < crop || g->rw < crop)
        return fail(VF_ERR_INVALID, "%s: a %dx%d frame resizes to %dx%d, smaller than the %d crop", who, H, W, g->rh,
                    g->rw, crop);
    g->resize = g->rh != H || g->rw != W;
    g->cy = center_crop_offset(g->rh, crop);
    g->cx = center_crop_offset(g->rw, crop);
    return VF_OK;
}

int resize_frames(EngineCore* h, const uint8_t* frames, int n, int H, int W, const FrameGeom& g, int max_frames,
                  cudaStream_t s, const uint8_t** src) {
    *src = frames;
    if (!g.resize) return VF_OK;
    VF_TRY(grow(h, &h->resized, &h->resized_cap, size_t(max_frames) * g.rh * g.rw * 3));
    VF_TRY(grow(h, &h->resize_tmp, &h->tmp_cap, size_t(max_frames) * H * g.rw * 3));
    VF_TRY(resize_u8(frames, n, H, W, h->resized, g.rh, g.rw, g.filter, h->resize_tmp, s));
    h->launches += (g.rh != H) + (g.rw != W);
    *src = h->resized;
    return VF_OK;
}

int balanced_step(int n, int max_frames) {
    const int nchunks = (n + max_frames - 1) / max_frames;
    return nchunks > 0 ? (n + nchunks - 1) / nchunks : max_frames;
}

int debug_frames(const EngineCore* h, const void* a, const void* b, int n, int limit, const char* limit_name,
                 const char* what) {
    if (!h || !a || !b) return fail(VF_ERR_INVALID, "%s: null argument", what);
    if (n <= 0 || n > limit)
        return fail(VF_ERR_INVALID, "%s: %d frames (1 .. %d, the handle's %s)", what, n, limit, limit_name);
    VF_CUDA(cudaSetDevice(h->device));
    return VF_OK;
}

GemmEpi linear_epi(void* out, int ldo, int out_f32, const float* bias, int act, int accumulate) {
    GemmEpi e;
    memset(&e, 0, sizeof(e));
    e.out = out; e.ldo = ldo; e.out_f32 = out_f32; e.bias = bias; e.act = act; e.accumulate = accumulate;
    return e;
}

}

using namespace vf;

extern "C" {

int vf_version(void) { return 2; }
const char* vf_last_error(void) { return g_err; }

int vf_sample_indices(const char* method, int param, int64_t frame_cnt, double fps, int64_t* out_idx, int64_t cap,
                      int64_t* out_n) {
    if (!method || !out_n) return fail(VF_ERR_INVALID, "sample_indices: null argument");
    int64_t n;
    if (strcmp(method, "uni") == 0) {
        n = param;
    } else if (strcmp(method, "fix") == 0) {
        volatile double t = double(frame_cnt) / fps;
        volatile double u = t * double(param);
        n = int64_t(u);
    } else {
        return fail(VF_ERR_UNSUPPORTED, "%s are not supported", method);
    }
    if (n < 0) return fail(VF_ERR_INVALID, "Number of samples, %lld, must be non-negative.", (long long)n);
    *out_n = n;
    if (n == 0 || out_idx == nullptr) return VF_OK;
    if (cap < n) return fail(VF_ERR_INVALID, "sample_indices: output capacity %lld < %lld",
                                         (long long)cap, (long long)n);
    const double start = 1.0, stop = double(frame_cnt - 2);
    if (n == 1) { out_idx[0] = int64_t(start); return VF_OK; }
    const double delta = stop - start;
    const double step = delta / double(n - 1);
    for (int64_t i = 0; i < n; ++i) {
        volatile double prod = (step == 0.0) ? (double(i) / double(n - 1)) * delta : double(i) * step;
        volatile double y = prod + start;
        out_idx[i] = int64_t(y);
    }
    out_idx[n - 1] = int64_t(stop);
    return VF_OK;
}

int vf_shard_range(int64_t n_items, int n_parts, int part, int64_t* begin, int64_t* end) {
    if (n_parts <= 0 || part < 0 || part >= n_parts || !begin || !end || n_items < 0)
        return fail(VF_ERR_INVALID, "shard_range: bad arguments");
    int64_t k = n_parts < n_items ? n_parts : n_items;
    if (k <= 0) { *begin = *end = 0; return VF_OK; }
    const int64_t cs = (n_items + k - 1) / k;
    int64_t b = int64_t(part) * cs, e = b + cs;
    if (b > n_items) b = n_items;
    if (e > n_items) e = n_items;
    *begin = b;
    *end = e;
    return VF_OK;
}

int vf_resize_geometry(int in_h, int in_w, int size, int to_smaller_edge, int* out_h, int* out_w) {
    if (in_h <= 0 || in_w <= 0 || size <= 0 || !out_h || !out_w) return fail(VF_ERR_INVALID, "resize_geometry");
    const int w = in_w, h = in_h;
    if ((w <= h && w == size) || (h <= w && h == size)) { *out_h = h; *out_w = w; return VF_OK; }
    if ((w < h) == (to_smaller_edge != 0)) { *out_w = size; *out_h = int(double(int64_t(size) * h) / double(w)); }
    else                                   { *out_h = size; *out_w = int(double(int64_t(size) * w) / double(h)); }
    return VF_OK;
}

int vf_resize_u8(const uint8_t* src, int n, int in_h, int in_w, uint8_t* dst, int out_h, int out_w, int filter,
                 uint8_t* tmp, void* stream) {
    if (!src || !dst) return fail(VF_ERR_INVALID, "resize: null buffer");
    return resize_u8(src, n, in_h, in_w, dst, out_h, out_w, filter, tmp, static_cast<cudaStream_t>(stream));
}

int vf_clip_normalize_u8(const uint8_t* src, int n, int src_h, int src_w, float* dst, void* stream) {
    if (!src || !dst) return fail(VF_ERR_INVALID, "clip_normalize: null buffer");
    if (src_h < 224 || src_w < 224) return fail(VF_ERR_INVALID, "clip_normalize: %dx%d smaller than the crop", src_h, src_w);
    if (n <= 0) return VF_OK;
    return launch_clip_normalize_f32(src, n, src_h, src_w, center_crop_offset(src_h, 224),
                                     center_crop_offset(src_w, 224), dst, static_cast<cudaStream_t>(stream));
}

int vf_gemm_profile(int enable) { return gemm_profile(enable); }
int vf_gemm_profile_read(double* ms, int64_t* launches, double* executed_flops) {
    return gemm_profile_read(ms, launches, executed_flops);
}

int vf_gemm_f16(const void* A, int lda, const void* B, int ldb, int M, int N, int K, void* D, int ldd, int out_f32,
                const float* bias, const float* scale, int act, void* stream) {
    if (!A || !B || !D) return fail(VF_ERR_INVALID, "gemm: null buffer");
    GemmEpi ep;
    memset(&ep, 0, sizeof(ep));
    ep.out = D; ep.ldo = ldd; ep.out_f32 = out_f32; ep.bias = bias; ep.scale = scale; ep.act = act;
    return gemm_f16(static_cast<const __half*>(A), lda, static_cast<const __half*>(B), ldb, M, N, K, ep,
                    static_cast<cudaStream_t>(stream));
}

int vf_gemm_f16_accumulate(const void* A, int lda, const void* B, int ldb, int M, int N, int K, float* D, int ldd,
                           const float* bias, const float* scale, int act, void* stream) {
    if (!A || !B || !D) return fail(VF_ERR_INVALID, "gemm: null buffer");
    GemmEpi ep;
    memset(&ep, 0, sizeof(ep));
    ep.out = D; ep.ldo = ldd; ep.out_f32 = 1; ep.bias = bias; ep.scale = scale; ep.act = act; ep.accumulate = 1;
    return gemm_f16(static_cast<const __half*>(A), lda, static_cast<const __half*>(B), ldb, M, N, K, ep,
                    static_cast<cudaStream_t>(stream));
}

int vf_gemm_f16_split(const void* A, int lda, const void* B, int ldb, int M, int N, int K, void* D, int ldd, int split_off,
                      const float* bias, const float* scale, int act, void* stream) {
    if (!A || !B || !D) return fail(VF_ERR_INVALID, "gemm: null buffer");
    if (split_off < N || ldd < split_off + N) return fail(VF_ERR_INVALID, "gemm: split output needs ldd >= split_off + N, split_off >= N");
    GemmEpi ep;
    memset(&ep, 0, sizeof(ep));
    ep.out = D; ep.ldo = ldd; ep.out_f32 = 0; ep.bias = bias; ep.scale = scale; ep.act = act; ep.split_off = split_off;
    return gemm_f16(static_cast<const __half*>(A), lda, static_cast<const __half*>(B), ldb, M, N, K, ep,
                    static_cast<cudaStream_t>(stream));
}

int vf_conv_gemm_f16(const void* X, int C, int64_t P, const void* Wt, int N, int ntaps, int k_per_tap, const int* tap_off,
                     int nsplit, uint64_t lo_mask, int row0, const int* region, void* D, int ldd, int out_f32, int split_off,
                     const float* bias, const float* scale, int act, void* stream) {
    if (!X || !Wt || !D || !tap_off) return fail(VF_ERR_INVALID, "conv_gemm: null buffer");
    if (ntaps < 1 || ntaps > 64) return fail(VF_ERR_INVALID, "conv_gemm: %d taps (1..64)", ntaps);
    if (split_off > 0 && ldd < split_off + N)
        return fail(VF_ERR_INVALID, "conv_gemm: split output needs ldd >= split_off + N");
    ConvGeom g;
    memset(&g, 0, sizeof(g));
    g.ntaps = ntaps; g.k_per_tap = k_per_tap; g.nsplit = nsplit; g.lo_mask = lo_mask; g.row0 = row0;
    memcpy(g.tap_off, tap_off, sizeof(int) * size_t(ntaps));
    if (region) {
        g.mask = 1;
        g.Tp = region[0]; g.Hp = region[1]; g.Wp = region[2];
        g.t0 = region[3]; g.t1 = region[4]; g.h0 = region[5]; g.h1 = region[6]; g.w0 = region[7]; g.w1 = region[8];
    }
    GemmEpi ep;
    memset(&ep, 0, sizeof(ep));
    ep.out = D; ep.ldo = ldd; ep.out_f32 = out_f32; ep.bias = bias; ep.scale = scale; ep.act = act; ep.split_off = split_off;
    return conv_gemm_f16(static_cast<const __half*>(X), C, P, static_cast<const __half*>(Wt), N, g, ep,
                         static_cast<cudaStream_t>(stream));
}

}
```

### video_features_b200/csrc/internal.h

```cpp
#pragma once
#include <cuda.h>
#include <cuda_runtime.h>
#include <cuda_fp16.h>
#include <stdint.h>
#include <stdio.h>

#include <array>
#include <functional>
#include <map>
#include <string>
#include <vector>

#include "../../include/vfeat.h"

namespace vf {

void set_error(const char* fmt, ...);
int fail(int code, const char* fmt, ...);

#define VF_CUDA(expr)                                                                       \
    do {                                                                                    \
        cudaError_t _e = (expr);                                                            \
        if (_e != cudaSuccess)                                                              \
            return vf::fail(VF_ERR_CUDA, "%s:%d: %s -> %s", __FILE__, __LINE__, #expr,      \
                            cudaGetErrorString(_e));                                        \
    } while (0)
#define VF_TRY(expr)                  \
    do {                              \
        int _s = (expr);              \
        if (_s != VF_OK) return _s;   \
    } while (0)

int check_device(int device);
bool graphs_enabled();
bool graph_trace();

using GraphKey = std::array<int, 4>;
struct CachedGraph {
    cudaGraphExec_t exec = nullptr;
    int64_t launches = 0;
};

struct EngineCore {
    const char* who = "";
    int device = 0;
    std::vector<void*> allocs;
    int64_t launches = 0;
    cudaStream_t cs = nullptr;
    cudaEvent_t ev_in = nullptr, ev_out = nullptr;
    bool use_graph = graphs_enabled();
    bool trace_graphs = graph_trace();
    std::map<GraphKey, CachedGraph> graphs;
    int capture_after = 1;
    size_t max_graphs = 16;
    bool evict_when_full = true;
    std::map<GraphKey, int> seen;
    uint8_t *resized = nullptr, *resize_tmp = nullptr;
    size_t resized_cap = 0, tmp_cap = 0;
};

int engine_alloc(EngineCore* h, void** p, size_t bytes);
template <typename Tp>
int ralloc(EngineCore* h, Tp** p, size_t count) {
    void* q = nullptr;
    VF_TRY(engine_alloc(h, &q, count * sizeof(Tp)));
    *p = static_cast<Tp*>(q);
    return VF_OK;
}
int open_stream(EngineCore* h);
int enter(EngineCore* h, cudaStream_t user);
int leave(EngineCore* h, cudaStream_t user);
void release(EngineCore* h);
int grow(EngineCore* h, uint8_t** p, size_t* cap, size_t need);
int upload_f32(EngineCore* h, float** dst, const float* src, size_t count);
int upload_f16(EngineCore* h, __half** dst, const float* src, size_t rows, size_t cols, size_t ld = 0,
               bool transpose = false);
int capture_graph(EngineCore* h, cudaStream_t s, const std::function<int()>& run, CachedGraph* g);
int run_graphed(EngineCore* h, const GraphKey& key, const std::function<int()>& run);

struct FrameGeom { int rh, rw, cy, cx; bool resize; int filter = VF_FILTER_BICUBIC; };
int frame_geometry(const char* who, int H, int W, int resize_to, int crop, FrameGeom* g);
int resize_frames(EngineCore* h, const uint8_t* frames, int n, int H, int W, const FrameGeom& g, int max_frames,
                  cudaStream_t s, const uint8_t** src);
int balanced_step(int n, int max_frames);
int debug_frames(const EngineCore* h, const void* a, const void* b, int n, int limit, const char* limit_name,
                 const char* what);

int make_tmap_2d(CUtensorMap* out, const void* base, int elem_bytes, uint64_t rows, uint64_t cols,
                 uint64_t row_pitch_bytes, uint32_t box_rows, uint32_t box_cols);

struct GemmEpi {
    void* out;
    const float* bias;
    const float* scale;
    int ldo;
    int out_f32;
    int act;
    int split_off;
    int accumulate;
};
GemmEpi linear_epi(void* out, int ldo, int out_f32, const float* bias, int act, int accumulate = 0);
int gemm_f16(const __half* A, int lda, const __half* B, int ldb, int M, int N, int K, const GemmEpi& ep,
             cudaStream_t stream);

struct ConvGeom {
    int ntaps;
    int k_per_tap;
    int tap_off[64];
    int nsplit;
    unsigned long long lo_mask;
    int row0;
    int mask;
    int Tp, Hp, Wp;
    int t0, t1, h0, h1, w0, w1;
};
int conv_gemm_f16(const __half* X, int C, int64_t P, const __half* Wt, int N, const ConvGeom& g, const GemmEpi& ep,
                  cudaStream_t stream);
int qkv_attention(const __half* h, int lda, const __half* w_perm, const float* bias_perm, __half* att, int n_frames, int heads,
                  cudaStream_t stream);
int device_sm_count();
int gemm_profile(int enable);
bool gemm_profile_on();
int gemm_profile_read(double* ms, int64_t* launches, double* flops);

int launch_clip_patchify(const uint8_t* src, int n, int src_h, int src_w, int crop_y, int crop_x, __half* patches,
                         int patch, cudaStream_t s);
int launch_clip_patchify_f32(const float* src_chw, int n, __half* patches, int patch, cudaStream_t s);
int launch_clip_normalize_f32(const uint8_t* src, int n, int src_h, int src_w, int crop_y, int crop_x, float* dst_chw,
                              cudaStream_t s);
int launch_add_layernorm(float* x, int64_t x_row_stride, const __half* y, int64_t y_row_stride, int write_x,
                         const float* gamma, const float* beta, void* out, int64_t out_row_stride, int out_f32, int rows,
                         cudaStream_t s);
int launch_embed_layernorm(const float* emb, const float* pos, const float* cls_pos0, const float* gamma,
                           const float* beta, float* x, int n_frames, int tokens, cudaStream_t s);
int launch_attention(const __half* qkv, __half* out, int n_frames, int tokens, int heads, cudaStream_t s);
int launch_resample(const uint8_t* src, int n, int in_h, int in_w, uint8_t* tmp, uint8_t* dst, int out_h, int out_w,
                    const int* kh_bounds, const int* kh_coef, int kh_size, const int* kv_bounds, const int* kv_coef,
                    int kv_size, cudaStream_t s);

int resize_u8(const uint8_t* src, int n, int in_h, int in_w, uint8_t* dst, int out_h, int out_w, int filter,
              uint8_t* tmp, cudaStream_t s);
int center_crop_offset(int dim, int crop);

}
```

Baseline: 46480.

## Add 128-row ping-pong GEMM tiles with wave-aware tile selection

Templates the warp-specialized GEMM kernel on BM so each ping-pong consumer warpgroup can issue two 64-row WGMMA fragments (128-row tiles), with producer and consumer register budgets adjusted for the larger accumulator. A new chooser picks (bm, bn) from a table by wave-quantized cost, breaking ties by traffic, replacing the bn-only heuristic. An explicit-tile API entry is also added. Larger tiles raise operand reuse per CTA for the CLIP linear layers, at the cost of register pressure, fewer pipeline stages, and extra template instantiations.

Measured after the change: 50800 (median of 6 runs). +9.3%, better.

```diff
diff --git a/include/vfeat.h b/include/vfeat.h
--- a/include/vfeat.h
+++ b/include/vfeat.h
@@ -43,6 +43,9 @@
                            const float* bias, const float* scale, int act, void* stream);
 int vf_gemm_f16_split(const void* A, int lda, const void* B, int ldb, int M, int N, int K, void* D, int ldd, int split_off,
                       const float* bias, const float* scale, int act, void* stream);
+int vf_gemm_f16_tile(const void* A, int lda, const void* B, int ldb, int M, int N, int K, void* D, int ldd, int out_f32,
+                     int split_off, int accumulate, const float* bias, const float* scale, int act, int bm, int bn,
+                     void* stream);
 int vf_conv_gemm_f16(const void* X, int C, int64_t P, const void* Wt, int N, int ntaps, int k_per_tap, const int* tap_off,
                      int nsplit, uint64_t lo_mask, int row0, const int* region, void* D, int ldd, int out_f32, int split_off,
                      const float* bias, const float* scale, int act, void* stream);
diff --git a/video_features_b200/_lib.py b/video_features_b200/_lib.py
--- a/video_features_b200/_lib.py
+++ b/video_features_b200/_lib.py
@@ -85,6 +85,9 @@
                                          C.c_int, C.c_void_p, C.c_void_p, C.c_int, C.c_void_p]),
     "vf_gemm_f16_split": (C.c_int, [C.c_void_p, C.c_int, C.c_void_p, C.c_int, C.c_int, C.c_int, C.c_int, C.c_void_p,
                                     C.c_int, C.c_int, C.c_void_p, C.c_void_p, C.c_int, C.c_void_p]),
+    "vf_gemm_f16_tile": (C.c_int, [C.c_void_p, C.c_int, C.c_void_p, C.c_int, C.c_int, C.c_int, C.c_int, C.c_void_p,
+                                   C.c_int, C.c_int, C.c_int, C.c_int, C.c_void_p, C.c_void_p, C.c_int, C.c_int, C.c_int,
+                                   C.c_void_p]),
     "vf_conv_gemm_f16": (C.c_int, [C.c_void_p, C.c_int, C.c_int64, C.c_void_p, C.c_int, C.c_int, C.c_int,
                                    C.POINTER(C.c_int), C.c_int, C.c_uint64, C.c_int, C.POINTER(C.c_int), C.c_void_p,
                                    C.c_int, C.c_int, C.c_int, C.c_void_p, C.c_void_p, C.c_int, C.c_void_p]),
diff --git a/video_features_b200/csrc/gemm.cu b/video_features_b200/csrc/gemm.cu
--- a/video_features_b200/csrc/gemm.cu
+++ b/video_features_b200/csrc/gemm.cu
@@ -69,20 +69,40 @@
 
 template <bool PP>
 static int run_gemm_launch(const CUtensorMap& tmA, const CUtensorMap& tmB, const CUtensorMap& tmD,
-                           const CUtensorMap& tmD2, int bn, const GemmEpi& ep, int M, int N, const ConvGeom& cg,
-                           cudaStream_t stream) {
+                           const CUtensorMap& tmD2, int bm, int bn, const GemmEpi& ep, int M, int N,
+                           const ConvGeom& cg, cudaStream_t stream) {
     const bool split = ep.split_off > 0 && !ep.out_f32;
     if constexpr (!PP) {
         if (cg.nsplit == 2)
-            return split ? launch_bn<2, true, PP>(tmA, tmB, tmD, tmD2, bn, ep, M, N, cg, stream)
-                         : launch_bn<2, false, PP>(tmA, tmB, tmD, tmD2, bn, ep, M, N, cg, stream);
-    }
-    return split ? launch_bn<1, true, PP>(tmA, tmB, tmD, tmD2, bn, ep, M, N, cg, stream)
-                 : launch_bn<1, false, PP>(tmA, tmB, tmD, tmD2, bn, ep, M, N, cg, stream);
-}
-
-static int run_gemm(const CUtensorMap& tmA, bool pp, const __half* B, int ldb, int64_t Ktot, int M, int N,
-                    const ConvGeom& cg, const GemmEpi& ep, cudaStream_t stream) {
+            return split ? launch_bn<2, true, PP>(tmA, tmB, tmD, tmD2, bm, bn, ep, M, N, cg, stream)
+                         : launch_bn<2, false, PP>(tmA, tmB, tmD, tmD2, bm, bn, ep, M, N, cg, stream);
+    }
+    return split ? launch_bn<1, true, PP>(tmA, tmB, tmD, tmD2, bm, bn, ep, M, N, cg, stream)
+                 : launch_bn<1, false, PP>(tmA, tmB, tmD, tmD2, bm, bn, ep, M, N, cg, stream);
+}
+
+static TileShape choose_tile(bool pp, int M, int N, int act, bool split) {
+    const int64_t sms = device_sm_count();
+    const TileShape* list = pp ? PP_TILES : COOP_TILES;
+    const int count = pp ? int(sizeof(PP_TILES) / sizeof(TileShape)) : int(sizeof(COOP_TILES) / sizeof(TileShape));
+    TileShape best = list[0];
+    int64_t best_cost = INT64_MAX, best_bytes = INT64_MAX;
+    for (int i = 0; i < count; ++i) {
+        const TileShape& t = list[i];
+        if (pp && !pp_tile_built(t, act, split)) continue;
+        const int64_t tiles = int64_t((M + t.bm - 1) / t.bm) * ((N + t.bn - 1) / t.bn);
+        const int64_t cost = (tiles + sms - 1) / sms * t.bm * t.bn, bytes = tiles * (t.bm + t.bn);
+        if (cost < best_cost || (cost == best_cost && bytes < best_bytes)) {
+            best = t;
+            best_cost = cost;
+            best_bytes = bytes;
+        }
+    }
+    return best;
+}
+
+static int run_gemm(const CUtensorMap& tmA, bool pp, TileShape tile, const __half* B, int ldb, int64_t Ktot, int M,
+                    int N, const ConvGeom& cg, const GemmEpi& ep, cudaStream_t stream) {
     if (!ep.out) return fail(VF_ERR_INVALID, "gemm: null output");
     if (reinterpret_cast<uintptr_t>(ep.out) & 15) return fail(VF_ERR_INVALID, "gemm: output must be 16-byte aligned");
     if (ep.accumulate && !ep.out_f32) return fail(VF_ERR_INVALID, "gemm: accumulate needs fp32 output");
@@ -91,14 +111,7 @@
     if (ep.out_f32 ? (ep.ldo % 4) : (ep.ldo % 8)) return fail(VF_ERR_INVALID, "gemm: ldo breaks 16-byte rows");
     if (ep.split_off && (ep.out_f32 || ep.split_off < N || ep.split_off % 8))
         return fail(VF_ERR_INVALID, "gemm: split output needs fp16 out and split_off >= N, multiple of 8");
-    const int bm = tile_rows(pp);
-    const int64_t num_m = (M + bm - 1) / bm, sms = device_sm_count();
-    int bn = 256;
-    int64_t best = INT64_MAX;
-    for (int cand : {256, 192, 128, 64}) {
-        const int64_t cost = (num_m * ((N + cand - 1) / cand) + sms - 1) / sms * cand;
-        if (cost < best) { best = cost; bn = cand; }
-    }
+    const int bm = tile.bm, bn = tile.bn;
     CUtensorMap tmB, tmD, tmD2;
     VF_TRY(make_tmap_2d(&tmB, B, 2, uint64_t(N), uint64_t(Ktot), uint64_t(ldb) * 2, uint32_t(bn), BK));
     const int eb = ep.out_f32 ? 4 : 2;
@@ -109,8 +122,8 @@
     else
         tmD2 = tmD;
     auto launch = [&] {
-        return pp ? run_gemm_launch<true>(tmA, tmB, tmD, tmD2, bn, ep, M, N, cg, stream)
-                  : run_gemm_launch<false>(tmA, tmB, tmD, tmD2, bn, ep, M, N, cg, stream);
+        return pp ? run_gemm_launch<true>(tmA, tmB, tmD, tmD2, bm, bn, ep, M, N, cg, stream)
+                  : run_gemm_launch<false>(tmA, tmB, tmD, tmD2, bm, bn, ep, M, N, cg, stream);
     };
     if (!g_prof.on) return launch();
     if (g_prof.used + 2 > g_prof.ev.size())
@@ -156,17 +169,27 @@
 }
 
 int gemm_f16(const __half* A, int lda, const __half* B, int ldb, int M, int N, int K, const GemmEpi& ep,
-             cudaStream_t stream) {
+             cudaStream_t stream, int bm, int bn) {
     if (M <= 0 || N <= 0 || K <= 0) return fail(VF_ERR_INVALID, "gemm: empty problem %dx%dx%d", M, N, K);
     if (K % 8 || lda % 8 || ldb % 8) return fail(VF_ERR_INVALID, "gemm: K/lda/ldb must be multiples of 8");
+    const bool split = ep.split_off > 0 && !ep.out_f32;
+    TileShape tile = choose_tile(true, M, N, ep.act, split);
+    if (bm || bn) {
+        bool built = false;
+        for (const TileShape& t : PP_TILES) built = built || (t.bm == bm && t.bn == bn && pp_tile_built(t, ep.act, split));
+        if (!built)
+            return fail(VF_ERR_INVALID, "gemm: no %dx%d tile is built for activation %d%s", bm, bn, ep.act,
+                        split ? " with split output" : "");
+        tile = TileShape{bm, bn};
+    }
     ConvGeom cg;
     memset(&cg, 0, sizeof(cg));
     cg.ntaps = 1;
     cg.k_per_tap = K;
     cg.nsplit = 1;
     CUtensorMap tmA;
-    VF_TRY(make_tmap_2d(&tmA, A, 2, uint64_t(M), uint64_t(K), uint64_t(lda) * 2, tile_rows(true), BK));
-    return run_gemm(tmA, true, B, ldb, K, M, N, cg, ep, stream);
+    VF_TRY(make_tmap_2d(&tmA, A, 2, uint64_t(M), uint64_t(K), uint64_t(lda) * 2, uint32_t(tile.bm), BK));
+    return run_gemm(tmA, true, tile, B, ldb, K, M, N, cg, ep, stream);
 }
 
 int conv_gemm_f16(const __half* X, int C, int64_t P, const __half* Wt, int N, const ConvGeom& g, const GemmEpi& ep,
@@ -182,10 +205,11 @@
     if (g.mask && (g.Tp < 1 || g.Hp < 1 || g.Wp < 1 || g.row0 < 0))
         return fail(VF_ERR_INVALID, "conv_gemm: bad mask volume %dx%dx%d, row0 %d", g.Tp, g.Hp, g.Wp, g.row0);
     CUtensorMap tmA;
-    VF_TRY(make_tmap_2d(&tmA, X, 2, uint64_t(P), uint64_t(g.k_per_tap), uint64_t(C) * 2, tile_rows(false), BK));
+    const TileShape tile = choose_tile(false, int(P), N, ep.act, false);
+    VF_TRY(make_tmap_2d(&tmA, X, 2, uint64_t(P), uint64_t(g.k_per_tap), uint64_t(C) * 2, uint32_t(tile.bm), BK));
     const int64_t Ktot = int64_t(g.ntaps) * g.k_per_tap * g.nsplit;
     if (Ktot % 8) return fail(VF_ERR_INVALID, "conv_gemm: K must be a multiple of 8");
-    return run_gemm(tmA, false, Wt, int(Ktot), Ktot, int(P), N, g, ep, stream);
-}
-
-}
+    return run_gemm(tmA, false, tile, Wt, int(Ktot), Ktot, int(P), N, g, ep, stream);
+}
+
+}
diff --git a/video_features_b200/csrc/gemm_kernel.cuh b/video_features_b200/csrc/gemm_kernel.cuh
--- a/video_features_b200/csrc/gemm_kernel.cuh
+++ b/video_features_b200/csrc/gemm_kernel.cuh
@@ -16,7 +16,6 @@
 
 constexpr int BK = 64;
 constexpr int THREADS = 384;
-constexpr uint32_t PRODUCER_REGS = 40, CONSUMER_REGS = 232;
 constexpr int EPI_ROWS = 64;
 constexpr uint32_t STG_BYTES = EPI_ROWS * 128;
 constexpr uint32_t STAGING_BYTES = 2 * 2 * STG_BYTES;
@@ -24,9 +23,11 @@
 constexpr uint32_t MAX_STAGES = 8;
 constexpr uint32_t RING_BUDGET = SMEM_LIMIT - STAGING_BYTES - 2 * MAX_STAGES * 8 - 1024;
 
-template <int BN, int NSPLIT, bool PP>
+template <int BM_, int BN, int NSPLIT, bool PP>
 struct GemmCfg {
-    static constexpr int BM = PP ? 64 : 128;
+    static constexpr int BM = BM_;
+    static constexpr int MT = PP ? BM / 64 : 1;
+    static constexpr uint32_t PRODUCER_REGS = MT == 2 ? 24 : 40, CONSUMER_REGS = MT == 2 ? 240 : 232;
     static constexpr uint32_t A_BYTES = BM * BK * 2;
     static constexpr uint32_t B_TILE = BN * BK * 2;
     static constexpr uint32_t B_BYTES = NSPLIT * B_TILE;
@@ -37,9 +38,8 @@
     static_assert(STAGES >= 2, "at least two pipeline stages");
     static_assert(SMEM_BYTES <= SMEM_LIMIT, "shared memory budget");
     static_assert(A_BYTES % 1024 == 0 && B_TILE % 1024 == 0, "swizzle-128B tiles must stay 1024-byte aligned");
+    static_assert(PP ? (BM == 64 || BM == 128) : BM == 128, "ping-pong tiles are 64 or 128 rows, cooperative 128");
 };
-
-constexpr int tile_rows(bool pp) { return pp ? GemmCfg<64, 1, true>::BM : GemmCfg<64, 1, false>::BM; }
 
 template <int ACT>
 __device__ __forceinline__ float apply_act(float v) {
@@ -59,15 +59,15 @@
     return v;
 }
 
-template <int BN, int NSPLIT, bool SPLIT, bool PP, int ACT>
+template <int BM, int BN, int NSPLIT, bool SPLIT, bool PP, int ACT>
 __global__ void __launch_bounds__(THREADS, 1)
 gemm_f16_kernel(const __grid_constant__ CUtensorMap tmA, const __grid_constant__ CUtensorMap tmB,
                 const __grid_constant__ CUtensorMap tmD, const __grid_constant__ CUtensorMap tmD2, const GemmEpi ep,
                 const int M, const int N, const __grid_constant__ ConvGeom cg) {
-    using Cfg = GemmCfg<BN, NSPLIT, PP>;
+    using Cfg = GemmCfg<BM, BN, NSPLIT, PP>;
     static_assert(PP ? NSPLIT == 1 : true, "split weights run in the conv mode only");
     constexpr int STAGES = Cfg::STAGES;
-    constexpr int BM = Cfg::BM;
+    constexpr int MT = Cfg::MT;
     extern __shared__ uint8_t smem_raw[];
     uint8_t* smem = reinterpret_cast<uint8_t*>((reinterpret_cast<uintptr_t>(smem_raw) + 1023) & ~uintptr_t(1023));
     uint8_t* sA = smem;
@@ -101,7 +101,7 @@
     __syncthreads();
 
     if (warp < 4) {
-        setmaxnreg_dec<PRODUCER_REGS>();
+        setmaxnreg_dec<Cfg::PRODUCER_REGS>();
         if (warp == 0 && lane == 0) {
             int stage = 0;
             uint32_t phase = 0;
@@ -128,11 +128,11 @@
         return;
     }
 
-    setmaxnreg_inc<CONSUMER_REGS>();
+    setmaxnreg_inc<Cfg::CONSUMER_REGS>();
     const int wg = (warp >> 2) - 1;
     const int wq = warp & 3;
     constexpr int R = BN / 2;
-    float acc[R];
+    float acc[MT * R];
     const bool issuer = (threadIdx.x & 127) == 0;
     uint32_t buf = 0;
     auto wg_sync = [&] {
@@ -172,16 +172,18 @@
             const uint64_t adesc = wgmma_desc_sw128(sA + stage * Cfg::A_BYTES + (PP ? 0 : wg * (64 * 128)));
             const uint64_t bdesc = wgmma_desc_sw128(sB + stage * Cfg::B_BYTES);
             const bool lo_blk = NSPLIT == 2 && ((cg.lo_mask >> kk) & 1ull);
-            wgmma_fence_regs<R>(acc);
+            wgmma_fence_regs<MT * R>(acc);
             wgmma_fence();
 #pragma unroll
             for (int k = 0; k < BK / 16; ++k) {
-                Wgmma<BN>::mma(acc, adesc + 2 * k, bdesc + 2 * k, (kb | k) != 0 ? 1u : 0u);
+#pragma unroll
+                for (int f = 0; f < MT; ++f)
+                    Wgmma<BN>::mma(acc + f * R, adesc + f * ((64 * 128) >> 4) + 2 * k, bdesc + 2 * k, (kb | k) != 0 ? 1u : 0u);
                 if (NSPLIT == 2 && !lo_blk) Wgmma<BN>::mma(acc, adesc + 2 * k, bdesc + (Cfg::B_TILE >> 4) + 2 * k, 1u);
             }
             wgmma_commit();
             wgmma_wait<1>();
-            wgmma_fence_regs<R>(acc);
+            wgmma_fence_regs<MT * R>(acc);
             if (prev >= 0) {
                 __syncwarp();
                 if (lane == 0) mbar_arrive(&empty[prev]);
@@ -192,50 +194,42 @@
         }
         if (PP && i + 1 < cta_tiles) pass_turn();
         float2 sc[8], bi[8];
+        auto load_sbc = [&](int s, int c) {
+            const int n = min(n0 + 64 * s + 8 * c + 2 * (lane & 3), N - 2);
+            sc[c] = ep.scale ? __ldg(reinterpret_cast<const float2*>(ep.scale + n)) : make_float2(1.f, 1.f);
+            bi[c] = ep.bias ? __ldg(reinterpret_cast<const float2*>(ep.bias + n)) : make_float2(-0.f, -0.f);
+        };
         auto load_sb = [&](int s) {
-#pragma unroll
-            for (int c = 0; c < 8; ++c) {
-                const int n = min(n0 + 64 * s + 8 * c + 2 * (lane & 3), N - 2);
-                sc[c] = ep.scale ? __ldg(reinterpret_cast<const float2*>(ep.scale + n)) : make_float2(1.f, 1.f);
-                bi[c] = ep.bias ? __ldg(reinterpret_cast<const float2*>(ep.bias + n)) : make_float2(-0.f, -0.f);
+            if (MT == 1) {
+#pragma unroll
+                for (int c = 0; c < 8; ++c) load_sbc(s, c);
             }
         };
         load_sb(0);
         wgmma_wait<0>();
-        wgmma_fence_regs<R>(acc);
+        wgmma_fence_regs<MT * R>(acc);
         __syncwarp();
         if (lane == 0) mbar_arrive(&empty[prev]);
 
-        bool keep[2] = {true, true};
-        if (cg.mask) {
-#pragma unroll
-            for (int h = 0; h < 2; ++h) {
-                const int mm = m0 + wq * 16 + (lane >> 2) + 8 * h - cg.row0;
-                const int w = mm % cg.Wp, r1 = mm / cg.Wp;
-                const int hh = r1 % cg.Hp, r2 = r1 / cg.Hp;
-                const int tt = r2 % cg.Tp;
-                keep[h] = (mm >= 0) && (w >= cg.w0) && (w < cg.w1) && (hh >= cg.h0) && (hh < cg.h1) && (tt >= cg.t0) && (tt < cg.t1);
-            }
-        }
-        const int row = m0;
+        bool keep[MT][2];
+#pragma unroll
+        for (int f = 0; f < MT; ++f) keep[f][0] = keep[f][1] = true;
+        if (!PP && cg.mask) {
+#pragma unroll
+            for (int f = 0; f < MT; ++f)
+#pragma unroll
+                for (int h = 0; h < 2; ++h) {
+                    const int mm = m0 + 64 * f + wq * 16 + (lane >> 2) + 8 * h - cg.row0;
+                    const int w = mm % cg.Wp, r1 = mm / cg.Wp;
+                    const int hh = r1 % cg.Hp, r2 = r1 / cg.Hp;
+                    const int tt = r2 % cg.Tp;
+                    keep[f][h] = (mm >= 0) && (w >= cg.w0) && (w < cg.w1) && (hh >= cg.h0) && (hh < cg.h1) && (tt >= cg.t0) && (tt < cg.t1);
+                }
+        }
         const uint32_t stg = smem_u32(sD) + wg * 2 * STG_BYTES + (wq * 16 + (lane >> 2)) * 128;
         const int swz = lane >> 2;
-#pragma unroll
-        for (int s = 0; s < BN / 64; ++s) {
-            if (n0 + 64 * s >= N) break;
-#pragma unroll
-            for (int c = 0; c < 8; ++c)
-#pragma unroll
-                for (int h = 0; h < 2; ++h) {
-                    const int j = 8 * s + c;
-                    float v0 = __fadd_rn(__fmul_rn(acc[4 * j + 2 * h], sc[c].x), bi[c].x);
-                    float v1 = __fadd_rn(__fmul_rn(acc[4 * j + 2 * h + 1], sc[c].y), bi[c].y);
-                    v0 = apply_act<ACT>(v0);
-                    v1 = apply_act<ACT>(v1);
-                    acc[4 * j + 2 * h] = keep[h] ? v0 : 0.f;
-                    acc[4 * j + 2 * h + 1] = keep[h] ? v1 : 0.f;
-                }
-            if (s + 1 < BN / 64) load_sb(s + 1);
+        auto store_box = [&](int s, int f) {
+            const int row = m0 + 64 * f;
             if (SPLIT) {
                 if (issuer) bulk_wait_read<0>();
                 wg_sync();
@@ -244,7 +238,7 @@
 #pragma unroll
                     for (int h = 0; h < 2; ++h) {
                         const int j = 8 * s + c;
-                        const float v0 = acc[4 * j + 2 * h], v1 = acc[4 * j + 2 * h + 1];
+                        const float v0 = acc[f * R + 4 * j + 2 * h], v1 = acc[f * R + 4 * j + 2 * h + 1];
                         const __half2 hi = __floats2half2_rn(v0, v1);
                         const uint32_t off = h * 8 * 128 + ((c ^ swz) << 4) + 4 * (lane & 3);
                         st_shared_b32(stg + off, *reinterpret_cast<const uint32_t*>(&hi));
@@ -268,8 +262,8 @@
                         const int chunk = 2 * c + ((lane & 3) >> 1);
 #pragma unroll
                         for (int h = 0; h < 2; ++h)
-                            st_shared_v2_f32(d + h * 8 * 128 + ((chunk ^ swz) << 4) + 8 * (lane & 1), acc[4 * j + 2 * h],
-                                             acc[4 * j + 2 * h + 1]);
+                            st_shared_v2_f32(d + h * 8 * 128 + ((chunk ^ swz) << 4) + 8 * (lane & 1),
+                                             acc[f * R + 4 * j + 2 * h], acc[f * R + 4 * j + 2 * h + 1]);
                     }
                     store_subtile(n0 + 64 * s + 32 * q, row);
                 }
@@ -281,74 +275,117 @@
                     for (int h = 0; h < 2; ++h) {
                         const int j = 8 * s + c;
                         st_shared_b32(d + h * 8 * 128 + ((c ^ swz) << 4) + 4 * (lane & 3),
-                                      pack_half2(acc[4 * j + 2 * h], acc[4 * j + 2 * h + 1]));
+                                      pack_half2(acc[f * R + 4 * j + 2 * h], acc[f * R + 4 * j + 2 * h + 1]));
                     }
                 store_subtile(n0 + 64 * s, row);
             }
+        };
+#pragma unroll
+        for (int s = 0; s < BN / 64; ++s) {
+            if (n0 + 64 * s >= N) break;
+#pragma unroll
+            for (int c = 0; c < 8; ++c) {
+                if (MT == 2) load_sbc(s, c);
+#pragma unroll
+                for (int f = 0; f < MT; ++f)
+#pragma unroll
+                    for (int h = 0; h < 2; ++h) {
+                        const int x = f * R + 4 * (8 * s + c) + 2 * h;
+                        float v0 = __fadd_rn(__fmul_rn(acc[x], sc[c].x), bi[c].x);
+                        float v1 = __fadd_rn(__fmul_rn(acc[x + 1], sc[c].y), bi[c].y);
+                        v0 = apply_act<ACT>(v0);
+                        v1 = apply_act<ACT>(v1);
+                        acc[x] = keep[f][h] ? v0 : 0.f;
+                        acc[x + 1] = keep[f][h] ? v1 : 0.f;
+                    }
+            }
+            if (s + 1 < BN / 64) load_sb(s + 1);
+            store_box(s, 0);
+            if (MT == 2 && m0 + 64 < M) store_box(s, 1);
         }
     }
     if (issuer) bulk_wait<0>();
 }
 
-template <int BN, int NSPLIT, bool SPLIT, bool PP, int ACT>
+template <int BM, int BN, int NSPLIT, bool SPLIT, bool PP, int ACT>
 int launch_gemm(const CUtensorMap& tmA, const CUtensorMap& tmB, const CUtensorMap& tmD, const CUtensorMap& tmD2,
                 const GemmEpi& ep, int M, int N, const ConvGeom& cg, cudaStream_t stream) {
-    using Cfg = GemmCfg<BN, NSPLIT, PP>;
+    using Cfg = GemmCfg<BM, BN, NSPLIT, PP>;
     static std::atomic<bool> attr_set[64];
     int dev = 0;
     VF_CUDA(cudaGetDevice(&dev));
     if (dev < 0 || dev >= 64 || !attr_set[dev].load(std::memory_order_acquire)) {
-        VF_CUDA(cudaFuncSetAttribute(gemm_f16_kernel<BN, NSPLIT, SPLIT, PP, ACT>,
+        VF_CUDA(cudaFuncSetAttribute(gemm_f16_kernel<BM, BN, NSPLIT, SPLIT, PP, ACT>,
                                      cudaFuncAttributeMaxDynamicSharedMemorySize, Cfg::SMEM_BYTES));
         if (dev >= 0 && dev < 64) attr_set[dev].store(true, std::memory_order_release);
     }
     const int tiles = ((M + Cfg::BM - 1) / Cfg::BM) * ((N + BN - 1) / BN);
     const int sms = device_sm_count();
     const int grid = tiles < sms ? tiles : sms;
-    gemm_f16_kernel<BN, NSPLIT, SPLIT, PP, ACT><<<grid, THREADS, Cfg::SMEM_BYTES, stream>>>(tmA, tmB, tmD, tmD2, ep, M,
-                                                                                            N, cg);
+    gemm_f16_kernel<BM, BN, NSPLIT, SPLIT, PP, ACT><<<grid, THREADS, Cfg::SMEM_BYTES, stream>>>(tmA, tmB, tmD, tmD2, ep,
+                                                                                                M, N, cg);
     VF_CUDA(cudaGetLastError());
     return VF_OK;
 }
 
-template <int BN, int NSPLIT, bool SPLIT, bool PP>
+template <int BM, int BN, int NSPLIT, bool SPLIT, bool PP>
 int launch_act(const CUtensorMap& tmA, const CUtensorMap& tmB, const CUtensorMap& tmD, const CUtensorMap& tmD2,
                const GemmEpi& ep, int M, int N, const ConvGeom& cg, cudaStream_t stream) {
-    switch (ep.act) {
-        case VF_ACT_QUICKGELU:
-            return launch_gemm<BN, NSPLIT, SPLIT, PP, VF_ACT_QUICKGELU>(tmA, tmB, tmD, tmD2, ep, M, N, cg, stream);
-        case VF_ACT_RELU:
-            return launch_gemm<BN, NSPLIT, SPLIT, PP, VF_ACT_RELU>(tmA, tmB, tmD, tmD2, ep, M, N, cg, stream);
-        case VF_ACT_SIGMOID:
-            return launch_gemm<BN, NSPLIT, SPLIT, PP, VF_ACT_SIGMOID>(tmA, tmB, tmD, tmD2, ep, M, N, cg, stream);
-        case VF_ACT_TANH:
-            return launch_gemm<BN, NSPLIT, SPLIT, PP, VF_ACT_TANH>(tmA, tmB, tmD, tmD2, ep, M, N, cg, stream);
-        case VF_ACT_LEAKY:
-            if constexpr (NSPLIT == 2 && !PP)
-                return launch_gemm<BN, NSPLIT, SPLIT, PP, VF_ACT_LEAKY>(tmA, tmB, tmD, tmD2, ep, M, N, cg, stream);
-            else
-                return fail(VF_ERR_INVALID, "gemm: LeakyReLU is built for split-weight convolutions (nsplit = 2) only");
-        case VF_ACT_GELU:
-            if constexpr (!SPLIT && ((NSPLIT == 1 && PP) || (NSPLIT == 2 && !PP)))
-                return launch_gemm<BN, NSPLIT, SPLIT, PP, VF_ACT_GELU>(tmA, tmB, tmD, tmD2, ep, M, N, cg, stream);
-            else
-                return fail(VF_ERR_INVALID, "gemm: GELU is built for gemm_f16 and split-weight convolutions, without split output, only");
-        default:
-            return launch_gemm<BN, NSPLIT, SPLIT, PP, VF_ACT_NONE>(tmA, tmB, tmD, tmD2, ep, M, N, cg, stream);
-    }
-}
-
+    if constexpr (PP && BM == 128 && BN == 192)
+        return launch_gemm<BM, BN, NSPLIT, SPLIT, PP, VF_ACT_NONE>(tmA, tmB, tmD, tmD2, ep, M, N, cg, stream);
+    else {
+        switch (ep.act) {
+            case VF_ACT_QUICKGELU:
+                return launch_gemm<BM, BN, NSPLIT, SPLIT, PP, VF_ACT_QUICKGELU>(tmA, tmB, tmD, tmD2, ep, M, N, cg, stream);
+            case VF_ACT_RELU:
+                return launch_gemm<BM, BN, NSPLIT, SPLIT, PP, VF_ACT_RELU>(tmA, tmB, tmD, tmD2, ep, M, N, cg, stream);
+            case VF_ACT_SIGMOID:
+                return launch_gemm<BM, BN, NSPLIT, SPLIT, PP, VF_ACT_SIGMOID>(tmA, tmB, tmD, tmD2, ep, M, N, cg, stream);
+            case VF_ACT_TANH:
+                return launch_gemm<BM, BN, NSPLIT, SPLIT, PP, VF_ACT_TANH>(tmA, tmB, tmD, tmD2, ep, M, N, cg, stream);
+            case VF_ACT_LEAKY:
+                if constexpr (NSPLIT == 2 && !PP)
+                    return launch_gemm<BM, BN, NSPLIT, SPLIT, PP, VF_ACT_LEAKY>(tmA, tmB, tmD, tmD2, ep, M, N, cg, stream);
+                else
+                    return fail(VF_ERR_INVALID, "gemm: LeakyReLU is built for split-weight convolutions (nsplit = 2) only");
+            case VF_ACT_GELU:
+                if constexpr (!SPLIT && ((NSPLIT == 1 && PP && BM == 64) || (NSPLIT == 2 && !PP)))
+                    return launch_gemm<BM, BN, NSPLIT, SPLIT, PP, VF_ACT_GELU>(tmA, tmB, tmD, tmD2, ep, M, N, cg, stream);
+                else
+                    return fail(VF_ERR_INVALID, "gemm: GELU is built for gemm_f16 and split-weight convolutions, without split output, only");
+            default:
+                return launch_gemm<BM, BN, NSPLIT, SPLIT, PP, VF_ACT_NONE>(tmA, tmB, tmD, tmD2, ep, M, N, cg, stream);
+        }
+    }
+}
+
+}
+
+struct TileShape {
+    int bm, bn;
+};
+constexpr TileShape PP_TILES[] = {{128, 192}, {128, 128}, {64, 256}, {64, 192}, {64, 128}, {64, 64}};
+constexpr TileShape COOP_TILES[] = {{128, 256}, {128, 192}, {128, 128}, {128, 64}};
+constexpr bool pp_tile_built(TileShape t, int act, bool split) {
+    return t.bm == 64 || (t.bn == 128 && act != VF_ACT_GELU) || (t.bn == 192 && act == VF_ACT_NONE && !split);
 }
 
 #define GEMM_LAUNCH_ARGS                                                                                           \
-    const CUtensorMap &tmA, const CUtensorMap &tmB, const CUtensorMap &tmD, const CUtensorMap &tmD2, int bn,       \
-        const GemmEpi &ep, int M, int N, const ConvGeom &cg, cudaStream_t stream
+    const CUtensorMap &tmA, const CUtensorMap &tmB, const CUtensorMap &tmD, const CUtensorMap &tmD2, int bm,       \
+        int bn, const GemmEpi &ep, int M, int N, const ConvGeom &cg, cudaStream_t stream
 template <int NSPLIT, bool SPLIT, bool PP>
 int launch_bn(GEMM_LAUNCH_ARGS) {
-    if (bn == 256) return launch_act<256, NSPLIT, SPLIT, PP>(tmA, tmB, tmD, tmD2, ep, M, N, cg, stream);
-    if (bn == 192) return launch_act<192, NSPLIT, SPLIT, PP>(tmA, tmB, tmD, tmD2, ep, M, N, cg, stream);
-    if (bn == 128) return launch_act<128, NSPLIT, SPLIT, PP>(tmA, tmB, tmD, tmD2, ep, M, N, cg, stream);
-    return launch_act<64, NSPLIT, SPLIT, PP>(tmA, tmB, tmD, tmD2, ep, M, N, cg, stream);
-}
-
-}
+    if constexpr (PP) {
+        if constexpr (!SPLIT) {
+            if (bm == 128 && bn == 192) return launch_act<128, 192, NSPLIT, SPLIT, PP>(tmA, tmB, tmD, tmD2, ep, M, N, cg, stream);
+        }
+        if (bm == 128) return launch_act<128, 128, NSPLIT, SPLIT, PP>(tmA, tmB, tmD, tmD2, ep, M, N, cg, stream);
+    }
+    constexpr int BM = PP ? 64 : 128;
+    if (bn == 256) return launch_act<BM, 256, NSPLIT, SPLIT, PP>(tmA, tmB, tmD, tmD2, ep, M, N, cg, stream);
+    if (bn == 192) return launch_act<BM, 192, NSPLIT, SPLIT, PP>(tmA, tmB, tmD, tmD2, ep, M, N, cg, stream);
+    if (bn == 128) return launch_act<BM, 128, NSPLIT, SPLIT, PP>(tmA, tmB, tmD, tmD2, ep, M, N, cg, stream);
+    return launch_act<BM, 64, NSPLIT, SPLIT, PP>(tmA, tmB, tmD, tmD2, ep, M, N, cg, stream);
+}
+
+}
diff --git a/video_features_b200/csrc/host.cu b/video_features_b200/csrc/host.cu
--- a/video_features_b200/csrc/host.cu
+++ b/video_features_b200/csrc/host.cu
@@ -437,6 +437,21 @@
                     static_cast<cudaStream_t>(stream));
 }
 
+int vf_gemm_f16_tile(const void* A, int lda, const void* B, int ldb, int M, int N, int K, void* D, int ldd, int out_f32,
+                     int split_off, int accumulate, const float* bias, const float* scale, int act, int bm, int bn,
+                     void* stream) {
+    if (!A || !B || !D) return fail(VF_ERR_INVALID, "gemm: null buffer");
+    if (bm == 0 || bn == 0) return fail(VF_ERR_INVALID, "gemm: the tile must be given (%dx%d)", bm, bn);
+    if (split_off && (split_off < N || ldd < split_off + N))
+        return fail(VF_ERR_INVALID, "gemm: split output needs ldd >= split_off + N, split_off >= N");
+    GemmEpi ep;
+    memset(&ep, 0, sizeof(ep));
+    ep.out = D; ep.ldo = ldd; ep.out_f32 = out_f32; ep.bias = bias; ep.scale = scale; ep.act = act;
+    ep.split_off = split_off; ep.accumulate = accumulate;
+    return gemm_f16(static_cast<const __half*>(A), lda, static_cast<const __half*>(B), ldb, M, N, K, ep,
+                    static_cast<cudaStream_t>(stream), bm, bn);
+}
+
 int vf_conv_gemm_f16(const void* X, int C, int64_t P, const void* Wt, int N, int ntaps, int k_per_tap, const int* tap_off,
                      int nsplit, uint64_t lo_mask, int row0, const int* region, void* D, int ldd, int out_f32, int split_off,
                      const float* bias, const float* scale, int act, void* stream) {
diff --git a/video_features_b200/csrc/internal.h b/video_features_b200/csrc/internal.h
--- a/video_features_b200/csrc/internal.h
+++ b/video_features_b200/csrc/internal.h
@@ -101,7 +101,7 @@
 };
 GemmEpi linear_epi(void* out, int ldo, int out_f32, const float* bias, int act, int accumulate = 0);
 int gemm_f16(const __half* A, int lda, const __half* B, int ldb, int M, int N, int K, const GemmEpi& ep,
-             cudaStream_t stream);
+             cudaStream_t stream, int bm = 0, int bn = 0);
 
 struct ConvGeom {
     int ntaps;
```
